# jbikker/tinybvh

Measured on AMD Instinct MI355X. Metric: MRays/s (primary + diffuse) on Bistro CWBVH, higher is better.
Workload: dtype f32; 1 GPU; procedural street (Bistro-exterior stand-in, 2.83M tris, seed 2); BVH8_CWBVH; per GPU per step 16777216 primary + 16777216 diffuse (depth 1-3) Intersect; scene_tris=2832120, layout=BVH8_CWBVH, scene_is_stand_in=True

## Files before the change

### include/tinybvh_amd.h

```cpp
#ifndef TINYBVH_AMD_H_
#define TINYBVH_AMD_H_

#include <stddef.h>
#include <stdint.h>

#ifdef __cplusplus
extern "C" {
#endif

#define TBVH_ABI_VERSION 5

#define TBVH_OK            0
#define TBVH_E_INVALID    -1
#define TBVH_E_NODEVICE   -2
#define TBVH_E_HIP        -3
#define TBVH_E_NOMEM      -4
#define TBVH_E_FORMAT     -5

#define TBVH_LAYOUT_BVH2_WALD  1
#define TBVH_LAYOUT_BVH_DOUBLE 3
#define TBVH_LAYOUT_BVH_GPU    5
#define TBVH_LAYOUT_BVH4_GPU   8
#define TBVH_LAYOUT_CWBVH     10
#define TBVH_LAYOUT_VOXELSET  12

typedef struct tbvh_context tbvh_context;
typedef struct tbvh_scene   tbvh_scene;
typedef struct tbvh_hostbvh tbvh_hostbvh;

int         tbvh_abi_version(void);
const char* tbvh_last_error(void);
int         tbvh_device_count(void);
int         tbvh_init(int device, tbvh_context** out);
void        tbvh_shutdown(tbvh_context* ctx);
int         tbvh_synchronize(tbvh_context* ctx);
int         tbvh_set_stream(tbvh_context* ctx, void* hip_stream);
int         tbvh_set_timing(tbvh_context* ctx, int enabled);


int tbvh_upload_bvh_gpu(tbvh_context* ctx, const void* nodes64, uint64_t n_nodes,
                        const uint32_t* prim_idx, uint64_t n_idx,
                        const void* verts16, uint64_t n_tris, tbvh_scene** out);

int tbvh_upload_bvh4_gpu(tbvh_context* ctx, const void* blocks16, uint64_t n_blocks,
                         tbvh_scene** out);

int tbvh_upload_cwbvh(tbvh_context* ctx, const void* nodes16, uint64_t n_node_blocks,
                      const void* tris16, uint64_t n_tri_blocks, tbvh_scene** out);

int tbvh_upload_tlas(tbvh_context* ctx, const void* tlas_nodes64, uint64_t n_nodes,
                     const uint32_t* tlas_idx, uint64_t n_idx,
                     const void* instances192, uint64_t n_instances,
                     tbvh_scene* const* blas, uint64_t n_blas, tbvh_scene** out);
int tbvh_update_tlas(tbvh_scene* tlas, const void* tlas_nodes64, uint64_t n_nodes,
                     const uint32_t* tlas_idx, uint64_t n_idx,
                     const void* instances192, uint64_t n_instances);

int tbvh_update_bvh_gpu(tbvh_scene* scene, const void* nodes64, uint64_t n_nodes, const uint32_t* prim_idx, uint64_t n_idx, const void* verts16, uint64_t n_tris);
int tbvh_update_bvh4_gpu(tbvh_scene* scene, const void* blocks16, uint64_t n_blocks);
int tbvh_update_cwbvh(tbvh_scene* scene, const void* nodes16, uint64_t n_node_blocks, const void* tris16, uint64_t n_tri_blocks);

int tbvh_convert_bvh2_device(tbvh_context* ctx, const void* nodes32, uint64_t n_nodes, const uint32_t* prim_idx, uint64_t n_idx,
                             const void* verts16, uint64_t n_tris, int on_device, int layout, tbvh_scene** out);

int tbvh_build_device(tbvh_context* ctx, const void* verts16, uint64_t n_tris, int on_device, int layout,
                      uint32_t max_leaf_tris, tbvh_scene** out);

int tbvh_build_device_ploc(tbvh_context* ctx, const void* verts16, uint64_t n_tris, int on_device, int layout, uint32_t radius, tbvh_scene** out);

int tbvh_scene_download(tbvh_scene* scene, int which, void* dst, uint64_t cap_bytes, uint64_t* bytes_out);

int tbvh_set_opacity_micromaps(tbvh_scene* blas, const uint32_t* map_data, uint32_t N, uint64_t n_tris, int on_device);

int tbvh_refit(tbvh_scene* scene, const void* verts16, uint64_t n_tris, int on_device);

int tbvh_rebuild_tlas_device(tbvh_scene* tlas, const void* transforms, int on_device,
                             const float* blas_bounds6, uint64_t n_blas);
int tbvh_tlas_download(tbvh_scene* tlas, void* tlas_nodes64, uint64_t cap_nodes, uint32_t* tlas_idx, uint64_t cap_idx,
                       void* instances192, uint64_t cap_instances, uint64_t* n_nodes_out);
void     tbvh_free_scene(tbvh_scene* scene);
int      tbvh_scene_layout(const tbvh_scene* scene);
uint64_t tbvh_scene_device_bytes(const tbvh_scene* scene);


int tbvh_intersect(tbvh_scene* scene, void* rays, uint64_t n_rays, uint32_t stride_bytes);
int tbvh_occluded(tbvh_scene* scene, const void* rays, uint64_t n_rays,
                  uint32_t stride_bytes, uint8_t* occluded);
int tbvh_pinned_malloc(tbvh_context* ctx, uint64_t bytes, void** out);
int tbvh_pinned_free(tbvh_context* ctx, void* ptr);

int tbvh_intersect_device(tbvh_scene* scene, void* d_rays64, uint64_t n_rays);
int tbvh_occluded_device(tbvh_scene* scene, const void* d_rays64, uint64_t n_rays,
                         uint8_t* d_occluded);
int tbvh_intersect_device_fresh(tbvh_scene* scene, void* d_rays64, uint64_t n_rays, float tmax);

int tbvh_intersect_sharded(tbvh_scene* const* scenes, uint32_t n_devices, void* rays, uint64_t n_rays, uint32_t stride_bytes);
int tbvh_occluded_sharded(tbvh_scene* const* scenes, uint32_t n_devices, const void* rays, uint64_t n_rays,
                          uint32_t stride_bytes, uint8_t* occluded);
int tbvh_intersect_sharded_device(tbvh_scene* const* scenes, uint32_t n_devices, void* const* d_rays64, const uint64_t* n_rays,
                                  int fresh, float tmax, float* kernel_ms, float* dispatch_ms);
int tbvh_occluded_sharded_device(tbvh_scene* const* scenes, uint32_t n_devices, const void* const* d_rays64, const uint64_t* n_rays,
                                 uint8_t* const* d_occluded, float* kernel_ms, float* dispatch_ms);
void tbvh_shard_range(uint64_t n_rays, uint32_t rank, uint32_t world, uint64_t* begin, uint64_t* end);

int tbvh_reset_hits_device(tbvh_context* ctx, void* d_rays64, uint64_t n_rays, float tmax);

float tbvh_time_last_ms(tbvh_context* ctx);

int tbvh_time_history(tbvh_context* ctx, float* ms, uint32_t cap, uint32_t* count);

int tbvh_measure_copy_bandwidth(tbvh_context* ctx, uint64_t bytes, uint32_t reps, double* gbps);
int tbvh_measure_read_bandwidth(tbvh_context* ctx, uint64_t bytes, uint32_t reps, double* gbps);
int tbvh_measure_valu_issue(tbvh_context* ctx, uint32_t reps, double* ginstr_per_s);
int tbvh_measure_link_bandwidth(tbvh_context* ctx, uint64_t bytes, uint32_t reps, double* h2d_gbps, double* d2h_gbps);

int tbvh_cwbvh_set_hybrid(tbvh_scene* scene, int64_t packed_nodes);

typedef struct tbvh_schedule_hint { uint8_t closest_hit[3]; uint8_t any_hit[3]; uint8_t reserved[2]; } tbvh_schedule_hint;
int tbvh_scene_get_schedule_hint(tbvh_scene* scene, tbvh_schedule_hint* out);
// ... 289 lines not shown
```

### include/tinybvh_amd_debug.h

```cpp
#ifndef TINYBVH_AMD_DEBUG_H_
#define TINYBVH_AMD_DEBUG_H_
#include "tinybvh_amd.h"
#ifdef __cplusplus
extern "C" {
#endif

int tbvh_debug_stats(tbvh_context* ctx, uint64_t out[8], int reset);

int tbvh_debug_set_flags(tbvh_context* ctx, uint32_t flags);

int tbvh_debug_coherent_schedule(tbvh_scene* scene, int anyhit, uint32_t out[4]);

int tbvh_debug_last_probe(tbvh_context* ctx, uint32_t out[3]);

int tbvh_set_variant(tbvh_scene* scene, int variant);

int tbvh_debug_wide_copy_bvh2(int layout, const void* blob, uint64_t n_blob, const uint32_t* prim_idx, uint64_t n_idx, const void* verts16, uint64_t n_tris,
                              uint32_t max_leaf_tris, void* nodes32_out, uint64_t cap_nodes, uint64_t* n_nodes_out, void* recs_out, uint64_t cap_recs,
                              uint64_t* n_recs_out);

int tbvh_debug_device_allocations(uint64_t out[2]);

struct tbvh_scenegraph;
int tbvh_debug_scenegraph_array(struct tbvh_scenegraph* g, int what, void** d_ptr);
int tbvh_debug_scenegraph_step(struct tbvh_scenegraph* g, int step, float dt);
struct tbvh_host_scenegraph;
int tbvh_debug_host_scenegraph_set_trs(struct tbvh_host_scenegraph* g, const float* trs10, uint64_t n_nodes);
int tbvh_debug_host_scenegraph_check_chains(struct tbvh_host_scenegraph* g, uint64_t* n_differ);

#ifdef __cplusplus
}
#endif
#endif
```

### tinybvh_amd/__init__.py

```python
from __future__ import annotations

import ctypes as C
from typing import Optional

import os

import numpy as np

from . import _capi
from ._capi import AlphaTexture, BuildParams, Camera, Mesh, OmmSource, TbvhError, check, lib

LAYOUT_BVH2_WALD = 1
LAYOUT_BVH_DOUBLE = 3
LAYOUT_BVH_GPU = 5
LAYOUT_BVH4_GPU = 8
LAYOUT_CWBVH = 10
LAYOUT_VOXELSET = 12
MATERIAL_DIFFUSE, MATERIAL_LIGHT, MATERIAL_SPECULAR = 0, 1, 2

BVH_FAR = np.float32(1e30)

RAY_DTYPE = np.dtype([
    ("O", "<f4", 3), ("mask", "<u4"),
    ("D", "<f4", 3), ("instIdx", "<u4"),
    ("rD", "<f4", 3), ("inst", "<u4"),
    ("t", "<f4"), ("u", "<f4"), ("v", "<f4"), ("prim", "<u4"),
])
assert RAY_DTYPE.itemsize == 64


def safercp(x: np.ndarray) -> np.ndarray:
    x = np.asarray(x, dtype=np.float32)
    big = np.abs(x) > np.float32(1e-12)
    with np.errstate(divide="ignore"):
        r = np.where(big, np.float32(1.0) / np.where(big, x, np.float32(1.0)), np.where(x >= 0, BVH_FAR, -BVH_FAR))
    return r.astype(np.float32)


def make_rays(O: np.ndarray, D: np.ndarray, tmax=BVH_FAR, normalize: bool = True) -> np.ndarray:
    O = np.ascontiguousarray(O, dtype=np.float32).reshape(-1, 3)
    D = np.ascontiguousarray(D, dtype=np.float32).reshape(-1, 3)
    if normalize:
        l = np.sqrt((D * D).sum(axis=1, dtype=np.float32)).astype(np.float32)
        rl = np.where(l == 0, np.float32(0), np.float32(1) / np.where(l == 0, np.float32(1), l)).astype(np.float32)
        D = (D * rl[:, None]).astype(np.float32)
    rays = np.zeros(O.shape[0], dtype=RAY_DTYPE)
    rays["O"] = O
    rays["D"] = D
    rays["rD"] = safercp(D)
    rays["mask"] = 0xFFFF
    rays["t"] = tmax
    return rays


def _ptr(a: np.ndarray) -> C.c_void_p:
    return C.c_void_p(a.ctypes.data)


class Context:

    def __init__(self, device: int = 0):
        h = C.c_void_p()
        check(lib.tbvh_init(device, C.byref(h)), "tbvh_init")
        self._h = h
        self.device = device

    def close(self):
        if self._h:
            lib.tbvh_shutdown(self._h)
            self._h = None

    def __del__(self):
        try:
            self.close()
        except Exception:
            pass

    def synchronize(self):
        check(lib.tbvh_synchronize(self._h), "tbvh_synchronize")

    def set_stream(self, hip_stream: Optional[int]):
        check(lib.tbvh_set_stream(self._h, C.c_void_p(hip_stream or 0)), "tbvh_set_stream")

    def set_timing(self, enabled: bool):
        check(lib.tbvh_set_timing(self._h, 1 if enabled else 0), "tbvh_set_timing")

    def copy_bandwidth_gbps(self, nbytes: int = 1 << 30, reps: int = 3) -> float:
        g = C.c_double(0)
        check(lib.tbvh_measure_copy_bandwidth(self._h, nbytes, reps, C.byref(g)), "tbvh_measure_copy_bandwidth")
        return float(g.value)

    def read_bandwidth_gbps(self, nbytes: int = 1 << 30, reps: int = 3) -> float:
        g = C.c_double(0)
        check(lib.tbvh_measure_read_bandwidth(self._h, nbytes, reps, C.byref(g)), "tbvh_measure_read_bandwidth")
        return float(g.value)

    def valu_issue_ginstr(self, reps: int = 3) -> float:
        g = C.c_double(0)
        check(lib.tbvh_measure_valu_issue(self._h, reps, C.byref(g)), "tbvh_measure_valu_issue")
        return float(g.value)

    def link_bandwidth_gbps(self, nbytes: int = 1 << 28, reps: int = 3):
        up, down = C.c_double(0), C.c_double(0)
        check(lib.tbvh_measure_link_bandwidth(self._h, nbytes, reps, C.byref(up), C.byref(down)), "tbvh_measure_link_bandwidth")
        return float(up.value), float(down.value)

    def pinned_array(self, shape, dtype) -> np.ndarray:
        dt = np.dtype(dtype)
        n = int(np.prod(shape)) * dt.itemsize
        p = C.c_void_p()
        check(lib.tbvh_pinned_malloc(self._h, max(n, 1), C.byref(p)), "tbvh_pinned_malloc")
        buf = (C.c_char * max(n, 1)).from_address(p.value)
        a = np.frombuffer(buf, dtype=dt, count=int(np.prod(shape))).reshape(shape)
        self._pinned = getattr(self, "_pinned", {})
        self._pinned[a.ctypes.data] = p.value
        return a

    def pinned_free(self, a: np.ndarray):
        p = getattr(self, "_pinned", {}).pop(a.ctypes.data, None)
        check(lib.tbvh_pinned_free(self._h, C.c_void_p(p if p is not None else a.ctypes.data)), "tbvh_pinned_free")

    def time_last_ms(self) -> float:
        return float(lib.tbvh_time_last_ms(self._h))

    def time_history(self, k: int):
        buf = (C.c_float * max(int(k), 1))()
        cnt = C.c_uint32(0)
        check(lib.tbvh_time_history(self._h, buf, int(k), C.byref(cnt)), "tbvh_time_history")
        return [float(buf[i]) for i in range(cnt.value)]

    def set_debug_flags(self, flags: int):
        check(lib.tbvh_debug_set_flags(self._h, int(flags)), "tbvh_debug_set_flags")

    def last_probe(self):
        out = (C.c_uint32 * 3)()
        check(lib.tbvh_debug_last_probe(self._h, out), "tbvh_debug_last_probe")
        return int(out[0]), int(out[1]), int(out[2])

    def malloc(self, nbytes: int) -> int:
        p = C.c_void_p()
        check(lib.tbvh_device_malloc(self._h, nbytes, C.byref(p)), "tbvh_device_malloc")
        return p.value

    def free(self, dptr: int):
        check(lib.tbvh_device_free(self._h, C.c_void_p(dptr)), "tbvh_device_free")

    def to_device(self, dptr: int, a: np.ndarray):
        a = np.ascontiguousarray(a)
        check(lib.tbvh_copy_to_device(self._h, C.c_void_p(dptr), _ptr(a), a.nbytes), "tbvh_copy_to_device")

    def from_device(self, a: np.ndarray, dptr: int):
        assert a.flags["C_CONTIGUOUS"]
        check(lib.tbvh_copy_from_device(self._h, _ptr(a), C.c_void_p(dptr), a.nbytes), "tbvh_copy_from_device")

    def flatten_mesh(self, verts, indices=None, d_out: int = 0) -> int:
        m, keep = _mesh(verts, indices)
        d = d_out or self.malloc(int(m.n_tris) * 48)
        check(lib.tbvh_flatten_mesh_device(self._h, C.byref(m), C.c_void_p(d)), "tbvh_flatten_mesh_device")
        return d

    def reset_hits(self, d_rays: int, n: int, tmax: float = 1e30):
        check(lib.tbvh_reset_hits_device(self._h, C.c_void_p(d_rays), n, float(tmax)), "tbvh_reset_hits_device")

    def generate_primary(self, cam: Camera, d_rays: int, first: int, n: int):
        check(lib.tbvh_generate_primary_device(self._h, C.byref(cam), C.c_void_p(d_rays), first, n), "tbvh_generate_primary_device")
# ... 1469 lines not shown
```

### tinybvh_amd/_capi.py

```python
from __future__ import annotations

import ctypes as C
import os

_HERE = os.path.dirname(os.path.abspath(__file__))
LIB_PATH = os.environ.get("TBVH_LIB_OVERRIDE") or os.path.join(_HERE, "libtinybvh_amd.so")

_u64, _u32, _vp, _i = C.c_uint64, C.c_uint32, C.c_void_p, C.c_int
_pp = C.POINTER(C.c_void_p)


class BuildParams(C.Structure):
    _fields_ = [("bins", _u32), ("max_leaf_tris", _u32), ("threads", _u32), ("flags", _u32)]


class Mesh(C.Structure):
    _fields_ = [("verts", C.c_void_p), ("n_verts", C.c_uint64), ("stride_bytes", C.c_uint32), ("on_device", C.c_uint32),
                ("indices", C.c_void_p), ("n_tris", C.c_uint64)]


class AlphaTexture(C.Structure):
    _fields_ = [("texels", C.c_void_p), ("width", C.c_uint32), ("height", C.c_uint32)]


class OmmSource(C.Structure):
    _fields_ = [("uv", C.c_void_p), ("n_uv", C.c_uint64), ("uv_stride_bytes", C.c_uint32), ("on_device", C.c_uint32), ("indices", C.c_void_p),
                ("n_tris", C.c_uint64), ("tri_texture", C.c_void_p), ("textures", C.POINTER(AlphaTexture)), ("n_textures", C.c_uint32)]


class SceneGraphDesc(C.Structure):
    _fields_ = [("flags", C.c_uint32), ("n_nodes", C.c_uint64), ("parent", C.c_void_p), ("visit_order", C.c_void_p), ("translation", C.c_void_p), ("rotation", C.c_void_p),
                ("scale", C.c_void_p), ("matrix", C.c_void_p), ("local_transform", C.c_void_p), ("n_weights", C.c_void_p), ("weights", C.c_void_p),
                ("n_samplers", C.c_uint64), ("sampler_interpolation", C.c_void_p), ("sampler_type", C.c_void_p), ("sampler_key_offset", C.c_void_p),
                ("sampler_value_offset", C.c_void_p), ("key_times", C.c_void_p), ("key_values", C.c_void_p), ("n_animations", C.c_uint64), ("n_channels", C.c_uint64),
                ("channel_animation", C.c_void_p), ("channel_sampler", C.c_void_p), ("channel_node", C.c_void_p), ("channel_target", C.c_void_p),
                ("n_instances", C.c_uint64), ("node_of_instance", C.c_void_p), ("n_skin_uses", C.c_uint64), ("skin_mesh_node", C.c_void_p),
                ("skin_joint_offset", C.c_void_p), ("skin_joint_node", C.c_void_p), ("skin_inverse_bind", C.c_void_p)]


class Camera(C.Structure):
    _fields_ = [("eye", C.c_float * 3), ("p1", C.c_float * 3), ("p2", C.c_float * 3), ("p3", C.c_float * 3),
                ("width", _u32), ("height", _u32), ("spp_x", _u32), ("spp_y", _u32)]


class WfParams(C.Structure):
    _fields_ = [("light_pos", C.c_float * 3), ("light_color", C.c_float * 3), ("sky_lo", C.c_float * 3), ("sky_hi", C.c_float * 3),
                ("eps", C.c_float), ("max_depth", _u32), ("seed", _u32), ("clear", _u32), ("light_size", C.c_float * 2), ("flags", _u32), ("sample_index", _u32)]


class WfStats(C.Structure):
    _fields_ = [("extend_rays", _u64 * 8), ("shadow_rays", _u64 * 8), ("frame_ms", C.c_float)]


SYMBOLS = {
    "tbvh_debug_wide_copy_bvh2": (_i, [_i, _vp, _u64, _vp, _u64, _vp, _u64, _u32, _vp, _u64, C.POINTER(_u64), _vp, _u64, C.POINTER(_u64)]),
    "tbvh_wavefront_create": (_i, [_vp, _u32, _u32, _pp]),
    "tbvh_wavefront_destroy": (None, [_vp]),
    "tbvh_wavefront_render": (_i, [_vp, _vp, _vp, C.POINTER(Camera), C.POINTER(WfParams), C.POINTER(WfStats)]),
    "tbvh_wavefront_read": (_i, [_vp, _vp]),
    "tbvh_wavefront_set_blas_vertices": (_i, [_vp, _vp, _u64]),
    "tbvh_wavefront_finalize": (_i, [_vp, C.c_float, _vp]),
    "tbvh_wavefront_set_blue_noise": (_i, [_vp, _vp, _u64]),
    "tbvh_abi_version": (_i, []),
    "tbvh_last_error": (C.c_char_p, []),
    "tbvh_device_count": (_i, []),
    "tbvh_init": (_i, [_i, _pp]),
    "tbvh_shutdown": (None, [_vp]),
    "tbvh_synchronize": (_i, [_vp]),
    "tbvh_set_stream": (_i, [_vp, _vp]),
    "tbvh_set_timing": (_i, [_vp, _i]),
    "tbvh_upload_bvh_gpu": (_i, [_vp, _vp, _u64, _vp, _u64, _vp, _u64, _pp]),
    "tbvh_upload_bvh4_gpu": (_i, [_vp, _vp, _u64, _pp]),
    "tbvh_upload_cwbvh": (_i, [_vp, _vp, _u64, _vp, _u64, _pp]),
    "tbvh_upload_tlas": (_i, [_vp, _vp, _u64, _vp, _u64, _vp, _u64, _pp, _u64, _pp]),
    "tbvh_update_tlas": (_i, [_vp, _vp, _u64, _vp, _u64, _vp, _u64]),
    "tbvh_update_bvh_gpu": (_i, [_vp, _vp, _u64, _vp, _u64, _vp, _u64]),
    "tbvh_update_bvh4_gpu": (_i, [_vp, _vp, _u64]),
    "tbvh_update_cwbvh": (_i, [_vp, _vp, _u64, _vp, _u64]),
    "tbvh_rebuild_tlas_device": (_i, [_vp, _vp, _i, _vp, _u64]),
    "tbvh_refit": (_i, [_vp, _vp, _u64, _i]),
    "tbvh_set_opacity_micromaps": (_i, [_vp, _vp, _u32, _u64, _i]),
    "tbvh_scene_download": (_i, [_vp, _i, _vp, _u64, _vp]),
    "tbvh_build_device": (_i, [_vp, _vp, _u64, _i, _i, _u32, _vp]),
    "tbvh_build_device_ploc": (_i, [_vp, _vp, _u64, _i, _i, _u32, _vp]),
    "tbvh_convert_bvh2_device": (_i, [_vp, _vp, _u64, _vp, _u64, _vp, _u64, _i, _i, _vp]),
    "tbvh_tlas_download": (_i, [_vp, _vp, _u64, _vp, _u64, _vp, _u64, _vp]),
    "tbvh_free_scene": (None, [_vp]),
    "tbvh_scene_layout": (_i, [_vp]),
    "tbvh_scene_device_bytes": (_u64, [_vp]),
    "tbvh_intersect": (_i, [_vp, _vp, _u64, _u32]),
    "tbvh_occluded": (_i, [_vp, _vp, _u64, _u32, _vp]),
    "tbvh_intersect_sharded": (_i, [_vp, _u32, _vp, _u64, _u32]),
    "tbvh_occluded_sharded": (_i, [_vp, _u32, _vp, _u64, _u32, _vp]),
    "tbvh_intersect_sharded_device": (_i, [_vp, _u32, _vp, _vp, _i, C.c_float, _vp, _vp]),
    "tbvh_occluded_sharded_device": (_i, [_vp, _u32, _vp, _vp, _vp, _vp, _vp]),
    "tbvh_wavefront_set_band": (_i, [_vp, _u32, _u32]),
    "tbvh_wavefront_render_sharded": (_i, [_vp, _vp, _vp, _u32, C.POINTER(Camera), _vp, _vp, _vp]),
    "tbvh_wavefront_read_sharded": (_i, [_vp, _u32, _vp]),
    "tbvh_shard_range": (None, [_u64, _u32, _u32, C.POINTER(_u64), C.POINTER(_u64)]),
    "tbvh_intersect_device": (_i, [_vp, _vp, _u64]),
    "tbvh_occluded_device": (_i, [_vp, _vp, _u64, _vp]),
    "tbvh_intersect_device_fresh": (_i, [_vp, _vp, _u64, C.c_float]),
    "tbvh_reset_hits_device": (_i, [_vp, _vp, _u64, C.c_float]),
    "tbvh_time_last_ms": (C.c_float, [_vp]),
    "tbvh_debug_coherent_schedule": (C.c_int, [_vp, C.c_int, C.POINTER(C.c_uint32)]),
    "tbvh_time_history": (C.c_int, [_vp, C.POINTER(C.c_float), C.c_uint32, C.POINTER(C.c_uint32)]),
    "tbvh_measure_copy_bandwidth": (_i, [_vp, _u64, _u32, C.POINTER(C.c_double)]),
    "tbvh_measure_read_bandwidth": (_i, [_vp, _u64, _u32, C.POINTER(C.c_double)]),
    "tbvh_measure_valu_issue": (_i, [_vp, _u32, C.POINTER(C.c_double)]),
    "tbvh_measure_link_bandwidth": (_i, [_vp, _u64, _u32, C.POINTER(C.c_double), C.POINTER(C.c_double)]),
    "tbvh_scene_get_schedule_hint": (_i, [_vp, _vp]),
    "tbvh_scene_set_schedule_hint": (_i, [_vp, _vp]),
    "tbvh_pinned_malloc": (_i, [_vp, _u64, _pp]),
    "tbvh_pinned_free": (_i, [_vp, _vp]),
    "tbvh_set_variant": (_i, [_vp, _i]),
    "tbvh_debug_stats": (_i, [_vp, _vp, _i]),
    "tbvh_debug_last_probe": (_i, [_vp, _vp]),
    "tbvh_debug_set_flags": (_i, [_vp, _u32]),
    "tbvh_debug_device_allocations": (_i, [C.POINTER(_u64)]),
    "tbvh_cwbvh_set_hybrid": (_i, [_vp, C.c_int64]),
    "tbvh_bin_rays_device": (_i, [_vp, _vp, _vp, _u64, C.POINTER(C.c_float), _u32, _u32, _vp]),
    "tbvh_generate_primary_device": (_i, [_vp, C.POINTER(Camera), _vp, _u64, _u64]),
    "tbvh_generate_bounce_device": (_i, [_vp, _vp, _vp, _vp, _u64, _u32]),
    "tbvh_generate_shadow_device": (_i, [_vp, _vp, _vp, _u64, C.POINTER(C.c_float), C.c_float]),
    "tbvh_device_malloc": (_i, [_vp, _u64, _pp]),
    "tbvh_device_free": (_i, [_vp, _vp]),
    "tbvh_copy_to_device": (_i, [_vp, _vp, _vp, _u64]),
    "tbvh_copy_from_device": (_i, [_vp, _vp, _vp, _u64]),
    "tbvh_host_build": (_i, [_vp, _u64, _i, C.POINTER(BuildParams), _pp]),
    "tbvh_host_build_tlas": (_i, [_vp, _u64, _vp, _u64, _pp]),
    "tbvh_host_free": (None, [_vp]),
    "tbvh_cwbvh_file_write": (_i, [C.c_char_p, _vp, _u64, _vp, _u64, _u64, _vp]),
    "tbvh_cwbvh_file_read": (_i, [C.c_char_p, _u64, _pp, C.POINTER(_u64)]),
    "tbvh_host_layout": (_i, [_vp]),
    "tbvh_host_blob": (_vp, [_vp, _i]),
    "tbvh_host_blob_count": (_u64, [_vp, _i]),
    "tbvh_upload_host": (_i, [_vp, _vp, _vp, _u64, _pp]),
    "tbvh_upload_bvh_double": (_i, [_vp, _vp, _u64, _vp, _u64, _vp, _u64, _pp]),
    "tbvh_upload_tlas_double": (_i, [_vp, _vp, _u64, _vp, _u64, _vp, _u64, _pp, _u64, _pp]),
    "tbvh_intersect_ex_device": (_i, [_vp, _vp, _u64]),
    "tbvh_occluded_ex_device": (_i, [_vp, _vp, _u64, _vp]),
    "tbvh_intersect_ex": (_i, [_vp, _vp, _u64]),
    "tbvh_occluded_ex": (_i, [_vp, _vp, _u64, _vp]),
    "tbvh_host_build_double": (_i, [_vp, _u64, _pp]),
    "tbvh_host_build_tlas_double": (_i, [_vp, _u64, _vp, _u64, _pp]),
    "tbvh_rebuild_tlas_double_device": (_i, [_vp, _vp, _i]),
    "tbvh_update_tlas_double": (_i, [_vp, _vp, _u64, _vp, _u64, _vp, _u64]),
    "tbvh_tlas_double_download": (_i, [_vp, _vp, _u64, _vp, _u64, _vp, _u64, _vp]),
    "tbvh_double_download": (_i, [_vp, _vp, _u64, _vp]),
    "tbvh_refit_double": (_i, [_vp, _vp, _u64, _i]),
    "tbvh_upload_voxelset": (_i, [_vp, _vp, _vp, _u64, _vp, _pp]),
    "tbvh_host_build_voxelset": (_i, [_vp, _u32, _u32, _u32, _pp]),
# ... 105 lines not shown
```

### tinybvh_amd/csrc/capi_context.hip

```cpp
#include "capi_internal.h"

using namespace tbvh;
using namespace tbvh_capi;

namespace {
thread_local char g_err[512] = "";
}

namespace tbvh_capi {
int fail(int code, const char* fmt, ...) {
    va_list ap;
    va_start(ap, fmt);
    vsnprintf(g_err, sizeof g_err, fmt, ap);
    va_end(ap);
    return code;
}

int setDevice(tbvh_context* c) {
    HIP_TRY(hipSetDevice(c->device));
    return 0;
}
hipError_t timedBegin(tbvh_context* c) {
    if (c->skipTiming) return hipSuccess;
    const uint32_t slot = (uint32_t)(c->evSeq % tbvh_context::kTimeRing);
    for (int k = 0; k < 2; k++)
        if (!c->evRing[slot][k]) { const hipError_t e = hipEventCreate(&c->evRing[slot][k]); if (e != hipSuccess) return e; }
    c->evDone[slot] = false;
    c->ev0 = c->evRing[slot][0]; c->ev1 = c->evRing[slot][1];
    c->evSeq++;
    return hipEventRecord(c->ev0, c->stream);
}
hipError_t timedEnd(tbvh_context* c) {
    if (c->skipTiming) return hipSuccess;
    const hipError_t e = hipEventRecord(c->ev1, c->stream);
    if (e == hipSuccess && c->evSeq) { c->evDone[(c->evSeq - 1) % tbvh_context::kTimeRing] = true; c->timed = true; }
    return e;
}
}

extern "C" {

int tbvh_abi_version(void) { return TBVH_ABI_VERSION; }
const char* tbvh_last_error(void) { return g_err; }

int tbvh_device_count(void) {
    int n = 0;
    hipError_t e = hipGetDeviceCount(&n);
    if (e != hipSuccess) { fail(TBVH_E_HIP, "hipGetDeviceCount: %s", hipGetErrorString(e)); return e == hipErrorNoDevice ? 0 : TBVH_E_HIP; }
    return n;
}

int tbvh_init(int device, tbvh_context** out) {
    if (!out) return fail(TBVH_E_INVALID, "tbvh_init: out is null");
    *out = nullptr;
    int n = 0;
    if (hipGetDeviceCount(&n) != hipSuccess || n <= 0) return fail(TBVH_E_NODEVICE, "no HIP device available");
    if (device < 0 || device >= n) return fail(TBVH_E_NODEVICE, "device %d out of range (0..%d)", device, n - 1);
    tbvh_context* c = new (std::nothrow) tbvh_context;
    if (!c) return fail(TBVH_E_NOMEM, "out of host memory");
    c->device = device;
    hipDeviceProp_t prop;
    hipError_t e = hipSetDevice(device);
    if (e == hipSuccess) e = hipGetDeviceProperties(&prop, device);
    if (e == hipSuccess) e = hipStreamCreateWithFlags(&c->ownStream, hipStreamNonBlocking);
    if (e != hipSuccess) { delete c; return fail(TBVH_E_HIP, "context setup failed: %s", hipGetErrorString(e)); }
    c->stream = c->ownStream;
    c->numCUs = prop.multiProcessorCount;
    c->blocks = (uint32_t)c->numCUs * 24u;
    if (const char* e = getenv("TBVH_BLOCKS_PER_CU")) {
        const int b = atoi(e);
        if (b >= 1 && b <= 32) { c->blocks = (uint32_t)c->numCUs * (uint32_t)b; c->gridOverride = true; }
    }
    if (const char* e = getenv("TBVH_RAYS_PER_BLOCK")) {
        const int b = atoi(e);
        if (b >= 64 && b <= 4096) { c->raysPerBlock = (uint32_t)b; c->gridOverride = true; }
    }
    if (const char* e = getenv("TBVH_SPLIT_RAYS")) { if (atoi(e) == 0) c->splitBelow = 0; }
    if (const char* e = getenv("TBVH_INCOHERENT_COPIES")) { if (atoi(e) == 0) c->incoherentCopies = false; }
    if (const char* e = getenv("TBVH_EMBED_TRIS")) { if (atoi(e) == 0) c->embedTris = false; }
    if (const char* e = getenv("TBVH_DEBUG_FLAGS")) c->expFlags = (uint32_t)strtoul(e, nullptr, 0);
    if (const char* e = getenv("TBVH_COHERENT_TUNER")) { const int v = atoi(e); c->cohTunerMode = v == 0 ? 1 : (v == 2 ? 2 : (v == 3 ? 3 : 0)); }
    if (const char* e = getenv("TBVH_POOL_PARTS")) {
        const int b = atoi(e);
        if (b >= 0 && (1 << b) <= kPoolParts) c->poolParts = (uint32_t)b;
    }
    c->spillEntries = 232;
    if (const char* e2 = getenv("TBVH_SPILL_ENTRIES")) {
        const int v = atoi(e2);
        if (v >= 2 && v <= 232) c->spillEntries = (uint32_t)v & ~1u;
    }
    const size_t spillBytes = (size_t)(c->blocks + c->blocks / 3u) * 64 * c->spillEntries * 4;
    e = c->spill.alloc(spillBytes / 4);
    if (e == hipSuccess) e = c->counter.alloc(32);
    if (e == hipSuccess) e = c->pool.alloc((size_t)(kPoolParts + 1) * kPoolCounterStride * 2);
    if (e != hipSuccess) { tbvh_shutdown(c); return fail(TBVH_E_NOMEM, "device allocation failed: %s", hipGetErrorString(e)); }
    c->status = (uint32_t*)(c->counter.get() + 4);
    hipMemset(c->counter, 0, 256);
    *out = c;
    return 0;
}

void tbvh_shutdown(tbvh_context* c) {
    if (!c) return;
    hipSetDevice(c->device);
    if (c->ownStream) hipStreamSynchronize(c->ownStream);
    for (;;) {
        tbvh_scene* t = nullptr;
        for (tbvh_scene* s : c->scenes) if (s->isTlas) { t = s; break; }
        if (!t) break;
        tbvh_free_scene(t);
    }
    while (!c->scenes.empty()) tbvh_free_scene(c->scenes.back());
    freePosesOf(c);
    freeGraphsOf(c);
    freeShadingsOf(c);
    freeOmmStagingOf(c);
    for (const tbvh_context::PinnedRange& r : c->pinned) hipHostFree(r.host);
    c->pinned.clear();
    delete c->pipe;
    for (auto& pair : c->evRing) for (hipEvent_t ev : pair) if (ev) hipEventDestroy(ev);
    if (c->ownStream) hipStreamDestroy(c->ownStream);
    delete c;
}

int tbvh_debug_device_allocations(uint64_t out[2]) {
    if (!out) return fail(TBVH_E_INVALID, "tbvh_debug_device_allocations: null argument");
    out[0] = g_devBufLive.load(); out[1] = g_devBufBytes.load();
    return 0;
}

int tbvh_synchronize(tbvh_context* c) {
    if (!c) return fail(TBVH_E_INVALID, "null context");
    TBVH_ENTER(c);
    HIP_TRY(hipStreamSynchronize(c->stream));
    return 0;
}

int tbvh_set_stream(tbvh_context* c, void* s) {
    if (!c) return fail(TBVH_E_INVALID, "null context");
    TBVH_LOCK(c);
    c->stream = s ? (hipStream_t)s : c->ownStream;
    return 0;
}

float tbvh_time_last_ms(tbvh_context* c) {
    if (!c) return -1.0f;
    TBVH_LOCK(c);
    if (!c->timed) return -1.0f;
    if (c->hostQuerySeq == c->evSeq && c->hostQueryMs >= 0.f) return c->hostQueryMs;
    hipSetDevice(c->device);
    if (hipEventSynchronize(c->ev1) != hipSuccess) return -1.0f;
    float ms = -1.0f;
    if (hipEventElapsedTime(&ms, c->ev0, c->ev1) != hipSuccess) return -1.0f;
    return ms;
}

int tbvh_time_history(tbvh_context* c, float* ms, uint32_t cap, uint32_t* count) {
    if (!c || !count || (!ms && cap)) return fail(TBVH_E_INVALID, "tbvh_time_history: null argument");
    *count = 0;
    TBVH_ENTER(c);
    uint64_t n = c->evSeq < tbvh_context::kTimeRing ? c->evSeq : tbvh_context::kTimeRing;
    if (n > cap) n = cap;
    for (uint64_t i = 0; i < n; i++) {
        const uint32_t slot = (uint32_t)((c->evSeq - n + i) % tbvh_context::kTimeRing);
        float t = -1.0f;
        if (c->evDone[slot]) {
            HIP_TRY(hipEventSynchronize(c->evRing[slot][1]));
            HIP_TRY(hipEventElapsedTime(&t, c->evRing[slot][0], c->evRing[slot][1]));
        }
        ms[i] = t;
    }
    *count = (uint32_t)n;
    return 0;
}

int tbvh_debug_stats(tbvh_context* c, uint64_t out[8], int reset) {
    if (!c || !out) return fail(TBVH_E_INVALID, "tbvh_debug_stats: null argument");
    TBVH_ENTER(c);
    HIP_TRY(hipStreamSynchronize(c->stream));
    HIP_TRY(hipMemcpy(out, c->counter + 8, 64, hipMemcpyDeviceToHost));
    if (reset) HIP_TRY(hipMemset(c->counter + 8, 0, 64));
    return 0;
}

int tbvh_set_timing(tbvh_context* c, int enabled) {
    if (!c) return fail(TBVH_E_INVALID, "tbvh_set_timing: null context");
    TBVH_LOCK(c);
    c->skipTiming = enabled == 0;
    return 0;
}

int tbvh_debug_set_flags(tbvh_context* c, uint32_t flags) {
    if (!c) return fail(TBVH_E_INVALID, "tbvh_debug_set_flags: null context");
    TBVH_LOCK(c);
    c->expFlags = flags;
    return 0;
}

int tbvh_debug_last_probe(tbvh_context* c, uint32_t out[3]) {
    if (!c || !out) return fail(TBVH_E_INVALID, "tbvh_debug_last_probe: null argument");
    TBVH_ENTER(c);
    out[0] = out[1] = out[2] = 0;
    if (!c->lastProbed) return 0;
    HIP_TRY(hipStreamSynchronize(c->stream));
    HIP_TRY(hipMemcpy(out, (uint32_t*)c->pool + (size_t)(c->poolCur ^ 1) * ((size_t)(kPoolParts + 1) * kPoolCounterStride) + (size_t)kPoolParts * kPoolCounterStride, 8, hipMemcpyDeviceToHost));
    out[2] = (out[1] != 0 && out[0] * 10u >= out[1] * 6u) ? 2u : 1u;
    return 0;
}


int tbvh_device_malloc(tbvh_context* c, uint64_t bytes, void** out) {
    if (!c || !out) return fail(TBVH_E_INVALID, "tbvh_device_malloc: null argument");
    TBVH_ENTER(c);
    hipError_t e = hipMalloc(out, bytes ? bytes : 16);
    if (e != hipSuccess) return fail(TBVH_E_NOMEM, "hipMalloc(%llu): %s", (unsigned long long)bytes, hipGetErrorString(e));
    return 0;
}
int tbvh_device_free(tbvh_context* c, void* p) {
    if (!c) return fail(TBVH_E_INVALID, "null context");
    TBVH_ENTER(c);
    HIP_TRY(hipStreamSynchronize(c->stream));
    HIP_TRY(hipFree(p));
    return 0;
}
int tbvh_copy_to_device(tbvh_context* c, void* d, const void* src, uint64_t bytes) {
    if (!c || ((!d || !src) && bytes)) return fail(TBVH_E_INVALID, "tbvh_copy_to_device: null argument");
    TBVH_ENTER(c);
    HIP_TRY(hipMemcpyAsync(d, src, bytes, hipMemcpyHostToDevice, c->stream));
    HIP_TRY(hipStreamSynchronize(c->stream));
    return 0;
}
int tbvh_copy_from_device(tbvh_context* c, void* dst, const void* d, uint64_t bytes) {
    if (!c || ((!d || !dst) && bytes)) return fail(TBVH_E_INVALID, "tbvh_copy_from_device: null argument");
    TBVH_ENTER(c);
    HIP_TRY(hipMemcpyAsync(dst, d, bytes, hipMemcpyDeviceToHost, c->stream));
    HIP_TRY(hipStreamSynchronize(c->stream));
    return 0;
}

static int timeBest(tbvh_context* c, uint32_t reps, const std::function<void()>& launch, double* bestMs) {
    hipEvent_t e0 = nullptr, e1 = nullptr;
    HIP_TRY(hipEventCreate(&e0));
    if (hipEventCreate(&e1) != hipSuccess) { hipEventDestroy(e0); return fail(TBVH_E_HIP, "hipEventCreate failed"); }
    double best = 0;
    hipError_t err = hipSuccess;
    for (uint32_t i = 0; i <= reps && err == hipSuccess; i++) {
        err = hipEventRecord(e0, c->stream);
        launch();
        if (err == hipSuccess) err = hipGetLastError();
        if (err == hipSuccess) err = hipEventRecord(e1, c->stream);
        if (err == hipSuccess) err = hipEventSynchronize(e1);
        float ms = 0;
        if (err == hipSuccess) err = hipEventElapsedTime(&ms, e0, e1);
        if (err == hipSuccess && i && ms > 0 && (best == 0 || ms < best)) best = ms;
    }
    hipEventDestroy(e0); hipEventDestroy(e1);
    if (err != hipSuccess) return fail(TBVH_E_HIP, "measurement launch failed: %s", hipGetErrorString(err));
    if (best <= 0) return fail(TBVH_E_HIP, "measurement produced no timing");
    *bestMs = best;
    return 0;
}

int tbvh_measure_copy_bandwidth(tbvh_context* c, uint64_t bytes, uint32_t reps, double* gbps) {
    if (!c || !gbps || bytes < (1u << 20)) return fail(TBVH_E_INVALID, "tbvh_measure_copy_bandwidth: null argument or under 1 MB");
    TBVH_ENTER(c);
    DevBuf<void> a, b;
    if (a.alloc(bytes) != hipSuccess || b.alloc(bytes) != hipSuccess) return fail(TBVH_E_NOMEM, "tbvh_measure_copy_bandwidth: cannot allocate 2 x %llu bytes", (unsigned long long)bytes);
    int r = 0;
    if (hipMemsetAsync(a, 1, bytes, c->stream) != hipSuccess) r = fail(TBVH_E_HIP, "hipMemsetAsync failed");
    double ms = 0;
    if (!r) r = timeBest(c, reps ? reps : 3, [&] { launch_stream_copy((const float4*)a.get(), (float4*)b.get(), bytes / 16, c->stream); }, &ms);
    if (r) return r;
    *gbps = 2.0 * (double)bytes / (ms * 1e-3) / 1e9;
    return 0;
}

int tbvh_measure_read_bandwidth(tbvh_context* c, uint64_t bytes, uint32_t reps, double* gbps) {
    if (!c || !gbps || bytes < (1u << 20)) return fail(TBVH_E_INVALID, "tbvh_measure_read_bandwidth: null argument or under 1 MB");
    TBVH_ENTER(c);
    DevBuf<void> a;
    DevBuf<float> sink;
    if (a.alloc(bytes) != hipSuccess || sink.alloc(64) != hipSuccess) return fail(TBVH_E_NOMEM, "tbvh_measure_read_bandwidth: cannot allocate %llu bytes", (unsigned long long)bytes);
    int r = 0;
    if (hipMemsetAsync(a, 1, bytes, c->stream) != hipSuccess) r = fail(TBVH_E_HIP, "hipMemsetAsync failed");
    double ms = 0;
    if (!r) r = timeBest(c, reps ? reps : 3, [&] { launch_stream_read((const float4*)a.get(), sink, bytes / 16, (uint32_t)c->numCUs * 32u, c->stream); }, &ms);
    if (r) return r;
    *gbps = (double)bytes / (ms * 1e-3) / 1e9;
// ... 36 lines not shown
```

### tinybvh_amd/csrc/capi_internal.h

```cpp
#pragma once
#include "../../include/tinybvh_amd.h"
#include "../../include/tinybvh_amd_debug.h"

#include <hip/hip_runtime.h>

#include <chrono>
#include <cmath>
#include <cstdarg>
#include <cstdio>
#include <cstdlib>
#include <cstring>
#include <new>
#include <atomic>
#include <condition_variable>
#include <functional>
#include <memory>
#include <mutex>
#include <string>
#include <thread>
#include <vector>

#include "copy_policy.h"
#include "dev_buf.h"
#include "host_builder.h"
#include "kernels.h"
#include "ray_pool.h"

using namespace tbvh;
using tbvh_capi::DevBuf;
using tbvh_capi::CopyKind;
using tbvh_capi::CopyPolicy;
using tbvh_capi::kCopyWide4;
using tbvh_capi::kCopyWide8;

static_assert(kLayoutBvhGpu == TBVH_LAYOUT_BVH_GPU && kLayoutBvh4Gpu == TBVH_LAYOUT_BVH4_GPU && kLayoutCwbvh == TBVH_LAYOUT_CWBVH,
              "kernels.h and the public header agree on the layout codes");

namespace tbvh_capi {
int fail(int code, const char* fmt, ...);
}

#define TBVH_REFUSE_DOUBLE(scene, who)                                                                                              \
    do {                                                                                                                            \
        if ((scene) && (scene)->layout == TBVH_LAYOUT_BVH_DOUBLE)                                                                   \
            return tbvh_capi::fail(TBVH_E_INVALID, "%s: a BVH_DOUBLE scene takes tbvh_intersect_ex / tbvh_occluded_ex only", who);   \
    } while (0)

#define TBVH_REFUSE_VOXEL(scene, who)                                                                                                   \
    do {                                                                                                                                \
        if ((scene) && (scene)->layout == TBVH_LAYOUT_VOXELSET)                                                                         \
            return tbvh_capi::fail(TBVH_E_INVALID, "%s: a VOXELSET scene takes the queries and can be a TLAS's BLAS; nothing else", who); \
    } while (0)

#define TBVH_REFUSE_CUSTOM(scene, who)                                                                                                    \
    do {                                                                                                                                  \
        if ((scene) && (scene)->layout == TBVH_LAYOUT_BVH2_WALD)                                                                          \
            return tbvh_capi::fail(TBVH_E_INVALID, "%s: a sphere BLAS (custom geometry) takes the queries and can be a TLAS's BLAS; nothing else", who); \
    } while (0)

#define HIP_TRY(expr)                                                                        \
    do {                                                                                     \
        hipError_t e_ = (expr);                                                              \
        if (e_ != hipSuccess) return fail(TBVH_E_HIP, "%s failed: %s", #expr, hipGetErrorString(e_)); \
    } while (0)

struct tbvh_context {
    std::recursive_mutex mu;
    int device = 0;
    hipStream_t ownStream = nullptr;
    hipStream_t stream = nullptr;
    static constexpr uint32_t kTimeRing = 256;
    hipEvent_t evRing[kTimeRing][2] = {};
    bool evDone[kTimeRing] = {};
    int cohTunerMode = 0;
    uint64_t evSeq = 0;
    hipEvent_t ev0 = nullptr, ev1 = nullptr;
    bool timed = false;
    int numCUs = 0;
    uint32_t blocks = 0;
    DevBuf<uint32_t> spill;
    uint32_t spillEntries = 0;
    DevBuf<unsigned long long> counter;
    uint32_t poolParts = 5;
    bool embedTris = true;
    bool incoherentCopies = true;
    uint32_t expFlags = 0;
    bool skipTiming = false;
    bool lastProbed = false;
    bool gridOverride = false;
    uint64_t splitBelow = 12ull << 20;
    uint32_t raysPerBlock = 128;
    DevBuf<uint32_t> pool;
    int poolCur = 0;
    bool poolClean = false;
    uint32_t* status = nullptr;
    DevBuf<RayRec> stageRays;
    DevBuf<uint8_t> stageOcc;
    struct HostPipe* pipe = nullptr;
    struct PinnedRange { char* host; uint64_t bytes; };
    float hostQueryMs = -1.f;
    uint64_t hostQuerySeq = ~0ull;
    std::vector<PinnedRange> pinned;
    DevBuf<void> binScratch;
    std::vector<tbvh_scene*> scenes;
    std::vector<struct tbvh_pose*> poses;
    std::vector<struct tbvh_scenegraph*> graphs;
    std::vector<struct tbvh_shading*> shadings;
    DevBuf<void> ommDesc;
    void* ommPin = nullptr;
    size_t ommPinBytes = 0;
    hipEvent_t ommEv = nullptr;
    bool ommPinUsed = false;
};

struct CohTuner {
    int decided = 0;
    bool pinned = false;
    uint32_t launches = 0;
    uint64_t refRays = 0;
    static constexpr int kModes = 3;
    uint32_t n[kModes] = {0, 0, 0};
    float best[kModes] = {1e30f, 1e30f, 1e30f};
    struct Pending { hipEvent_t e0, e1; int mode; uint64_t rays; };
    std::vector<Pending> pending;
    static constexpr uint32_t kSamples = 3;
    void drop_pending() { for (Pending& p : pending) { hipEventDestroy(p.e0); hipEventDestroy(p.e1); } pending.clear(); }
    void harvest(float minMs);
    void settle(bool packetOrStrict, float margin);
    int least_sampled() const;
};

struct WideCopies {
    tbvh_scene* copy8 = nullptr;
    tbvh_scene* copy4 = nullptr;
    bool tried8 = false, tried4 = false;
    bool tlasOnly = false;
    CopyPolicy policy;
    uint8_t live() const { return (uint8_t)((copy8 ? kCopyWide8 : 0) | (copy4 ? kCopyWide4 : 0)); }
    uint8_t pending() const { return policy.pendingCopies; }
};

struct CwbvhLayouts {
    DevBuf<float4> padded;
    DevBuf<float4> hybrid;
    DevBuf<uint32_t> perm;
    DevBuf<float4> trisPadded;
    uint32_t packed = 0;
    bool tried = false;
    bool levelOrder = false;
};

struct tbvh_scene {
    tbvh_context* ctx = nullptr;
    int layout = 0;
    int variant = 0;
    DevBuf<float4> nodes;
    DevBuf<float4> tris;
    CwbvhLayouts cw;
    CohTuner cohTuner[2][4];
    uint8_t cohLastClass[2] = {2, 2};
    uint32_t nNodes = 0;
    uint64_t nNodeBlocks = 0, nTriBlocks = 0;
    uint64_t capNodeBlocks = 0, capTriBlocks = 0;
    uint64_t topoHash = 0;
    uint64_t bytes = 0;
    bool isTlas = false;
    DevBuf<uint32_t> tlasIdx;
    DevBuf<float4> instances;
    DevBuf<BlasDesc> blasDesc;
    int blasLayout = 0;
    bool blasMixCw2 = false;
    bool blasSpheres = false;
    DevBuf<BlasDesc> blasDescAny;
    bool anyHitSeen = false;
    int blasLayoutAny = -1;
    bool blasMixCw2Any = false;
    uint64_t nInst = 0, nBlas = 0, nTlasNodes = 0, nTlasIdx = 0;
    DevBuf<float4> tlas4;
// ... 30 lines not shown
    uint64_t dblTris = 0, dblRecs = 0;
    uint32_t dblLeaves = 0;
};

struct BLASInstanceCheck { float m[32]; float mn[3]; uint32_t blasIdx; float mx[3]; uint32_t mask; uint32_t pad[8]; };
static_assert(sizeof(BLASInstanceCheck) == 192, "BLASInstance is 192 bytes");

struct tbvh_hostbvh {
    int layout = 0;
    BVH2 bvh2;
    std::vector<NodeAL> al;
    std::vector<Vec4> blocksA, blocksB;
    std::vector<NodeDbl> dnodes;
    std::vector<uint64_t> didx;
    std::vector<uint32_t> vgrid, vbricks, vtop;
};

struct HostPipe {
    static constexpr uint64_t kChunk = 1ull << 18;
    void* pinUp[2] = {nullptr, nullptr};
    hipEvent_t evUp[2] = {nullptr, nullptr};
    hipStream_t down = nullptr;
    hipEvent_t evKernel = nullptr;
    std::vector<hipEvent_t> evGroup;
    DevBuf<uint32_t> packed;
    void* pinDown = nullptr;
    std::vector<std::thread> workers;
    std::mutex m;
    std::condition_variable cvWork, cvDone;
    std::function<void(uint32_t, uint32_t)> job;
    uint64_t generation = 0;
    uint32_t pending = 0;
    bool quit = false;
    void start(uint32_t nThreads) {
        for (uint32_t t = 0; t < nThreads; t++)
            workers.emplace_back([this, t, nThreads] {
                uint64_t seen = 0;
                for (;;) {
                    std::function<void(uint32_t, uint32_t)> f;
                    {
                        std::unique_lock<std::mutex> lk(m);
                        cvWork.wait(lk, [&] { return quit || generation != seen; });
                        if (quit) return;
                        seen = generation; f = job;
                    }
                    f(t + 1, nThreads + 1);
                    {
                        std::lock_guard<std::mutex> lk(m);
                        if (--pending == 0) cvDone.notify_all();
                    }
                }
            });
    }
    void parallel_for(uint64_t items, const std::function<void(uint32_t, uint32_t)>& f) {
        if (items < 16384 || workers.empty()) { f(0, 1); return; }
        {
            std::lock_guard<std::mutex> lk(m);
            job = f; pending = (uint32_t)workers.size(); generation++;
        }
        cvWork.notify_all();
        f(0, (uint32_t)workers.size() + 1);
        std::unique_lock<std::mutex> lk(m);
        cvDone.wait(lk, [&] { return pending == 0; });
    }
    ~HostPipe() {
        { std::lock_guard<std::mutex> lk(m); quit = true; }
        cvWork.notify_all();
        for (auto& w : workers) w.join();
        for (int i = 0; i < 2; i++) {
            if (pinUp[i]) hipHostFree(pinUp[i]);
            if (evUp[i]) hipEventDestroy(evUp[i]);
        }
        for (hipEvent_t e : evGroup) hipEventDestroy(e);
        if (evKernel) hipEventDestroy(evKernel);
        if (down) hipStreamDestroy(down);
        if (pinDown) hipHostFree(pinDown);
    }
};

namespace tbvh_capi {
int setDevice(tbvh_context* c);
#define TBVH_LOCK(ctxptr) std::lock_guard<std::recursive_mutex> ctx_lock_((ctxptr)->mu)
#define TBVH_ENTER(ctxptr) std::lock_guard<std::recursive_mutex> ctx_lock_((ctxptr)->mu); if (int r_ = tbvh_capi::setDevice(ctxptr)) return r_
hipError_t timedBegin(tbvh_context* c);
hipError_t timedEnd(tbvh_context* c);
int launchQuery(tbvh_scene* s, tbvh::RayRec* d_rays, uint64_t n, uint8_t* d_occ, bool fresh = false, float freshTmax = 1e30f,
                const unsigned long long* nDev = nullptr);
int checkStatus(tbvh_context* c);
int ensureStage(tbvh_context* c, uint64_t n);
int ensureStageOcc(tbvh_context* c, uint64_t n);
tbvh_scene* newScene(tbvh_context* c, int layout);
int reclassifyTlas(tbvh_scene* t);
uint64_t cwbvhTopologyHash(const tbvh::Vec4* nodes, uint32_t nNodes);
int prepareIncoherentCopies(tbvh_scene* s);
int rederiveCwbvhLayouts(tbvh_scene* s);
int resetCwbvhLayouts(tbvh_scene* s, bool levelOrder = false);
void freeCopy(tbvh_scene* s, CopyKind kind);
void makeCopyOnce(tbvh_scene* b, CopyKind kind);
void dropCopiesAfterUpdate(tbvh_scene* s);
void countQueryForRecopy(tbvh_scene* s);
tbvh_scene* wideCopyForQuery(tbvh_scene* s);
tbvh_scene* tunedScene(tbvh_scene* s);
void shareOpacityMaps(tbvh_scene* s);
int refitCopies(tbvh_scene* s, const tbvh::MeshSrc& src);
const tbvh_scene* blasView(const tbvh_scene* b, bool any, bool allow4 = true);
template <class F>
int forEachTlasOver(tbvh_scene* b, F f) {
    for (size_t i = 0; i < b->usedBy.size(); i++) {
        bool seen = false;
        for (size_t k = 0; k < i; k++) seen |= b->usedBy[k] == b->usedBy[i];
        if (!seen) if (int r = f(b->usedBy[i])) return r;
    }
    return 0;
}
int checkMesh(const tbvh_mesh* m, const char* who, bool indicesMayBeHeld = false);
tbvh_mesh flatMesh(const void* verts16, uint64_t nTris, int onDevice);
uint64_t meshVertexBytes(const tbvh_mesh& m);
struct DeviceMesh {
    tbvh::MeshSrc src;
    DevBuf<void> ownVerts;
    DevBuf<uint32_t> ownIdx;
};
int stageMesh(tbvh_context* c, const tbvh_mesh& m, DeviceMesh& out);
int keepMeshIndices(tbvh_scene* s, const tbvh::MeshSrc& src);
int convertDeviceImpl(tbvh_context* c, int layout, const float4* dN2, uint64_t nNodes2, const uint32_t* dIdx, uint64_t nIdx, const tbvh::MeshSrc& dV, tbvh_scene** out);
int refitDeviceSource(tbvh_scene* s, const tbvh::MeshSrc& src);
int hostBuildImpl(const tbvh::HostMesh& mesh, uint64_t nTris, int layout, const tbvh_build_params* p, tbvh_hostbvh** out);
int checkSphereScene(tbvh_scene* s, const char* who);
int launchSpheres(tbvh_scene* s, const float4* dSpheres, uint64_t n, const tbvh::MeshSrc& verts, uint8_t* dHit);
int allocOpacityMaps(tbvh_context* c, uint32_t N, uint64_t nTris, const char* who, DevBuf<uint32_t>& fresh, uint64_t* wordsOut);
int installOpacityMaps(tbvh_scene* s, DevBuf<uint32_t>&& fresh, uint32_t N);
void freeOmmStagingOf(tbvh_context* c);
void freeGraphsOf(tbvh_context* c);
void freePosesOf(tbvh_context* c);
void freeShadingsOf(tbvh_context* c);
tbvh_context* shadingContext(const struct tbvh_shading* sh);
void shadingSlotRecords(const struct tbvh_shading* sh, uint32_t slot, float4** tris, uint64_t* nTris);
void detachPosesFrom(tbvh_context* c, const struct tbvh_shading* sh);
}
```

### tinybvh_amd/csrc/capi_pose.hip

```cpp
#include "capi_internal.h"
#include "pose.h"

using namespace tbvh;
using namespace tbvh_capi;

struct tbvh_pose {
    tbvh_context* ctx = nullptr;
    int kind = 0;
    uint64_t nVerts = 0;
    uint32_t nJoints = 0, nTargets = 0;
    DevBuf<float4> rest, weights;
    DevBuf<uint4> joints;
    DevBuf<float> positions;
    DevBuf<float> params;
    DevBuf<float4> out;
    tbvh_shading* shading = nullptr;
    uint32_t slot = 0;
    uint64_t fatTris = 0;
    DevBuf<float> normals;
    DevBuf<float4> nOut;
    DevBuf<uint32_t> fatIdx;
    char* pin = nullptr;
    uint64_t pinSlotBytes = 0;
    hipEvent_t pinEv[2] = {nullptr, nullptr};
// ... 151 lines not shown
    if (nTargets != p->nTargets) return fail(TBVH_E_INVALID, "tbvh_pose_set_morph: %u weights, the pose was created with %u targets", nTargets, p->nTargets);
    if (nTargets && !weights) return fail(TBVH_E_INVALID, "tbvh_pose_set_morph: null weights");
    if (onDevice && ((uintptr_t)weights & 3)) return fail(TBVH_E_INVALID, "tbvh_pose_set_morph: device weights must be 4-byte aligned");
    tbvh_context* c = p->ctx;
    TBVH_ENTER(c);
    float4* fat = nullptr;
    if (int r = attachedRecords(p, "tbvh_pose_set_morph", &fat)) return r;
    const float* dW = nullptr;
    if (int r = stageParams(p, weights, (uint64_t)nTargets * 4, onDevice, &dW)) return r;
    HIP_TRY(timedBegin(c));
    if (p->shading) {
        launch_pose_morph_normals(p->positions, nTargets ? dW : p->params.get(), nTargets, p->normals, p->out, p->nOut, p->nVerts, c->stream);
        updateFatTris(p, fat);
    } else
        launch_pose_morph(p->positions, nTargets ? dW : p->params.get(), nTargets, p->out, p->nVerts, c->stream);
    HIP_TRY(hipGetLastError());
    HIP_TRY(timedEnd(c));
    return 0;
}

int tbvh_pose_attach_fat_tris(tbvh_pose* p, tbvh_shading* sh, uint32_t slot, const float* normals12, const uint32_t* indices, uint64_t nTris, int onDevice) {
    if (!p || !sh || !normals12) return fail(TBVH_E_INVALID, "tbvh_pose_attach_fat_tris: null argument");
    if (shadingContext(sh) != p->ctx) return fail(TBVH_E_INVALID, "tbvh_pose_attach_fat_tris: the pose and the shading table belong to different contexts");
    if (((uintptr_t)normals12 | (uintptr_t)indices) & 3) return fail(TBVH_E_INVALID, "tbvh_pose_attach_fat_tris: misaligned normals or indices (4 bytes)");
    if (nTris == 0 || nTris >> 32) return fail(TBVH_E_INVALID, "tbvh_pose_attach_fat_tris: %llu triangles", (unsigned long long)nTris);
    if (!indices && p->nVerts != 3 * nTris)
        return fail(TBVH_E_INVALID, "tbvh_pose_attach_fat_tris: %llu vertices for %llu triangles: without indices triangle i has corners 3i .. 3i + 2", (unsigned long long)p->nVerts, (unsigned long long)nTris);
    tbvh_context* c = p->ctx;
    TBVH_ENTER(c);
    float4* tris = nullptr; uint64_t have = 0;
    shadingSlotRecords(sh, slot, &tris, &have);
    if (have != nTris) return fail(TBVH_E_INVALID, "tbvh_pose_attach_fat_tris: slot %u of the shading table holds %llu records, not %llu", slot, (unsigned long long)have, (unsigned long long)nTris);
    if (indices && !onDevice) {
        const uint64_t bad = pose_first_bad_corner(indices, nTris, p->nVerts);
        if (bad != nTris) return fail(TBVH_E_FORMAT, "tbvh_pose_attach_fat_tris: triangle %llu: an index is not a vertex (%llu vertices)", (unsigned long long)bad, (unsigned long long)p->nVerts);
    }
    const uint64_t nFloats = (p->kind == kPoseMorph ? (uint64_t)p->nTargets + 1 : 1) * p->nVerts * 3;
    DevBuf<float> normals; DevBuf<float4> nOut; DevBuf<uint32_t> idx;
    if (normals.alloc(nFloats) != hipSuccess || nOut.alloc(p->nVerts) != hipSuccess || (indices && idx.alloc(3 * nTris) != hipSuccess))
        return allocFail("tbvh_pose_attach_fat_tris", nFloats * 4 + p->nVerts * 16 + (indices ? nTris * 12 : 0));
    const hipMemcpyKind kind = onDevice ? hipMemcpyDeviceToDevice : hipMemcpyHostToDevice;
    HIP_TRY(hipMemcpyAsync(normals, normals12, nFloats * 4, kind, c->stream));
    if (indices) HIP_TRY(hipMemcpyAsync(idx, indices, nTris * 12, kind, c->stream));
    HIP_TRY(hipStreamSynchronize(c->stream));
    p->normals = std::move(normals); p->nOut = std::move(nOut); p->fatIdx = std::move(idx);
    p->shading = sh; p->slot = slot; p->fatTris = nTris;
    return 0;
}

int tbvh_pose_vertices(tbvh_pose* p, const void** dVerts16, uint64_t* nVerts) {
    if (!p || !dVerts16) return fail(TBVH_E_INVALID, "tbvh_pose_vertices: null argument");
    TBVH_LOCK(p->ctx);
    *dVerts16 = p->out.get();
    if (nVerts) *nVerts = p->nVerts;
    return 0;
}

int tbvh_pose_refit(tbvh_pose* p, tbvh_scene* s) {
    if (!p || !s) return fail(TBVH_E_INVALID, "tbvh_pose_refit: null argument");
    if (s->ctx != p->ctx) return fail(TBVH_E_INVALID, "tbvh_pose_refit: the pose and the scene belong to different contexts");
    TBVH_ENTER(p->ctx);
    if (s->meshIdx) {
        tbvh_mesh m;
        m.verts = p->out.get(); m.n_verts = p->nVerts; m.stride_bytes = 16; m.on_device = 1; m.indices = nullptr; m.n_tris = s->meshIdxTris;
        return tbvh_refit_mesh(s, &m);
    }
    if (p->nVerts % 3) return fail(TBVH_E_INVALID, "tbvh_pose_refit: %llu vertices: a scene without an index buffer takes 3 per triangle", (unsigned long long)p->nVerts);
    return tbvh_refit(s, p->out.get(), p->nVerts / 3, 1);
}

int tbvh_pose_download(tbvh_pose* p, void* dst16, uint64_t capVerts) {
    if (!p || !dst16) return fail(TBVH_E_INVALID, "tbvh_pose_download: null argument");
    if (capVerts < p->nVerts) return fail(TBVH_E_INVALID, "tbvh_pose_download: room for %llu vertices, the pose has %llu", (unsigned long long)capVerts, (unsigned long long)p->nVerts);
    tbvh_context* c = p->ctx;
    TBVH_ENTER(c);
    HIP_TRY(hipMemcpyAsync(dst16, p->out, p->nVerts * 16, hipMemcpyDeviceToHost, c->stream));
    return checkStatus(c);
}

void tbvh_pose_free(tbvh_pose* p) {
    if (!p) return;
    tbvh_context* c = p->ctx;
    TBVH_LOCK(c);
    hipSetDevice(c->device);
    hipStreamSynchronize(c->stream);
    for (size_t i = 0; i < c->poses.size(); i++)
        if (c->poses[i] == p) { c->poses.erase(c->poses.begin() + i); break; }
    destroyPose(p);
}

}
```

### tinybvh_amd/csrc/capi_query.hip

```cpp
#include "capi_internal.h"

using namespace tbvh;
using namespace tbvh_capi;

namespace tbvh_capi {
int ensureStage(tbvh_context* c, uint64_t n) {
    HIP_TRY(c->stageRays.reserve(n));
    return 0;
}
int ensureStageOcc(tbvh_context* c, uint64_t n) {
    HIP_TRY(c->stageOcc.reserve(n));
    return 0;
}
}

void CohTuner::harvest(float minMs) {
    for (size_t k = 0; k < pending.size();) {
        const Pending pe = pending[k];
        const hipError_t qe = hipEventQuery(pe.e1);
        if (qe == hipErrorNotReady) { (void)hipGetLastError(); k++; continue; }
        float t1 = 0.f;
        if (qe == hipSuccess && hipEventElapsedTime(&t1, pe.e0, pe.e1) == hipSuccess && t1 > minMs) {
            if (!refRays) refRays = pe.rays;
            if (pe.rays * 4 >= refRays * 3 && pe.rays * 3 <= refRays * 4) {
// ... 69 lines not shown
constexpr uint64_t kDirectRays = 16384;

static int hostQuerySmall(tbvh_scene* s, const char* raysIn, char* raysOut, uint64_t n, uint32_t stride, uint8_t* occ) {
    tbvh_context* c = s->ctx;
    if (int r = ensureStage(c, n)) return r;
    if (occ) if (int r = ensureStageOcc(c, n)) return r;
    HIP_TRY(hipMemcpy2DAsync(c->stageRays, 64, raysIn, stride, 64, n, hipMemcpyHostToDevice, c->stream));
    if (int r = launchQuery(s, c->stageRays, n, occ ? c->stageOcc : nullptr)) return r;
    if (occ) HIP_TRY(hipMemcpyAsync(occ, c->stageOcc, n, hipMemcpyDeviceToHost, c->stream));
    else HIP_TRY(hipMemcpy2DAsync(raysOut + 44, stride, (const char*)c->stageRays.get() + 44, 64, 20, n, hipMemcpyDeviceToHost, c->stream));
    return checkStatus(c);
}

int hostQuery(tbvh_scene* s, const char* raysIn, char* raysOut, uint64_t n, uint32_t stride, uint8_t* occ) {
    tbvh_context* c = s->ctx;
    if (n <= kDirectRays) return hostQuerySmall(s, raysIn, raysOut, n, stride, occ);
    if (int r = ensureStage(c, n)) return r;
    if (occ) if (int r = ensureStageOcc(c, n)) return r;
    const uint64_t G = n <= kGroupRays + kGroupRays / 2 ? 1 : (n + kGroupRays - 1) / kGroupRays;
    const uint64_t per = (((n + G - 1) / G) + HostPipe::kChunk - 1) / HostPipe::kChunk * HostPipe::kChunk;
    if (int r = ensurePipe(c, occ ? (n + 19) / 20 : 2 * per)) return r;
    HostPipe* p = c->pipe;
    const bool direct = stride == 64 && isPinned(c, raysIn, n * 64);
    while (p->evGroup.size() < G) { hipEvent_t e = nullptr; HIP_TRY(hipEventCreateWithFlags(&e, hipEventDisableTiming)); p->evGroup.push_back(e); }
    const uint64_t seq0 = c->evSeq;
    uint64_t chunkNo = 0;
    auto drain = [&](uint64_t g) -> int {
        const uint64_t b = g * per, e = b + per < n ? b + per : n;
        HIP_TRY(hipEventSynchronize(p->evGroup[g]));
        const char* pin = (const char*)p->pinDown + (g & 1) * per * 20;
        p->parallel_for(e - b, [=](uint32_t part, uint32_t parts) {
            const uint64_t lo = (e - b) * part / parts, hi = (e - b) * (part + 1) / parts;
            for (uint64_t i = lo; i < hi; i++) std::memcpy(raysOut + (b + i) * stride + 44, pin + i * 20, 20);
        });
        return 0;
    };
    for (uint64_t g = 0; g < G; g++) {
        const uint64_t b = g * per, e = b + per < n ? b + per : n;
        for (uint64_t first = b; first < e; first += HostPipe::kChunk, chunkNo++) {
            const uint64_t cnt = e - first < HostPipe::kChunk ? e - first : HostPipe::kChunk;
            if (direct) { HIP_TRY(hipMemcpyAsync(c->stageRays + first, raysIn + first * 64, cnt * 64, hipMemcpyHostToDevice, c->stream)); continue; }
            const int k = (int)(chunkNo & 1);
            if (chunkNo >= 2) HIP_TRY(hipEventSynchronize(p->evUp[k]));
            char* pin = (char*)p->pinUp[k];
            const char* src = raysIn + first * stride;
            p->parallel_for(cnt, [=](uint32_t part, uint32_t parts) {
                const uint64_t lo = cnt * part / parts, hi = cnt * (part + 1) / parts;
                if (stride == 64) std::memcpy(pin + lo * 64, src + lo * 64, (hi - lo) * 64);
                else for (uint64_t i = lo; i < hi; i++) std::memcpy(pin + i * 64, src + i * stride, 64);
            });
            HIP_TRY(hipMemcpyAsync(c->stageRays + first, pin, cnt * 64, hipMemcpyHostToDevice, c->stream));
            HIP_TRY(hipEventRecord(p->evUp[k], c->stream));
        }
        if (int r = launchQuery(s, c->stageRays + b, e - b, occ ? c->stageOcc + b : nullptr)) return r;
        if (!occ) {
            uint32_t* packed = p->packed + (g & 1) * per * 5;
            HIP_TRY(hipEventRecord(p->evKernel, c->stream));
            HIP_TRY(hipStreamWaitEvent(p->down, p->evKernel, 0));
            launch_pack_hits(c->stageRays + b, packed, e - b, p->down);
            HIP_TRY(hipGetLastError());
            HIP_TRY(hipMemcpyAsync((char*)p->pinDown + (g & 1) * per * 20, packed, (e - b) * 20, hipMemcpyDeviceToHost, p->down));
            HIP_TRY(hipEventRecord(p->evGroup[g], p->down));
            if (g) if (int r = drain(g - 1)) return r;
        }
    }
    if (occ) HIP_TRY(hipMemcpyAsync(p->pinDown, c->stageOcc, n, hipMemcpyDeviceToHost, c->stream));
    else if (int r = drain(G - 1)) return r;
    if (int r = checkStatus(c)) return r;
    if (occ) std::memcpy(occ, p->pinDown, n);
    if (!c->skipTiming && c->evSeq - seq0 == G && G <= tbvh_context::kTimeRing) {
        float sum = 0.f; bool ok = true;
        for (uint64_t q = seq0; q < c->evSeq && ok; q++) {
            const uint32_t slot = (uint32_t)(q % tbvh_context::kTimeRing);
            float t = 0.f;
            ok = c->evDone[slot] && hipEventElapsedTime(&t, c->evRing[slot][0], c->evRing[slot][1]) == hipSuccess;
            sum += t;
        }
        if (ok) { c->hostQueryMs = sum; c->hostQuerySeq = c->evSeq; } else (void)hipGetLastError();
    }
    return 0;
}


static void launchTlasKernels(tbvh_scene* s, QueryArgs& q, bool any, uint32_t blocks) {
    tbvh_context* c = s->ctx;
    const uint32_t blocks7 = (!c->gridOverride && blocks == c->blocks) ? (uint32_t)c->numCUs * 28u : blocks;
    const bool own = any && s->blasDescAny != nullptr;
    const int layout = own ? s->blasLayoutAny : s->blasLayout;
    const bool mix = own ? s->blasMixCw2Any : s->blasMixCw2;
    const BlasDesc* desc = own ? s->blasDescAny : s->blasDesc;
    if (s->blasSpheres) {
        q.spillStride = c->spillEntries / 2;
        launch_tlas_custom(any, layout, s->nodes, s->tlasIdx, s->instances, desc, q, c->status, blocks, c->stream);
    } else if (s->tlas4 && layout == TBVH_LAYOUT_BVH4_GPU) {
        q.spillStride = c->spillEntries;
        launch_tlas4(any, 0, s->tlas4, s->instances, desc, q, c->status, blocks, c->stream, blocks7);
    } else if (s->tlas8 && (layout == TBVH_LAYOUT_CWBVH || mix)) {
        q.spillStride = c->spillEntries / 2;
        launch_tlas8(any, 0, s->tlas8, s->tlas8Refs, s->instances, desc, q, c->status, blocks, c->stream, blocks7, mix);
    } else if (layout == TBVH_LAYOUT_VOXELSET) {
        q.spillStride = c->spillEntries;
        launch_voxel(any, nullptr, s->nodes, s->tlasIdx, s->instances, desc, q, c->status, blocks, c->stream);
    } else if (layout == TBVH_LAYOUT_BVH_GPU) {
        q.spillStride = c->spillEntries;
        launch_tlas2(any, 0, s->nodes, s->tlasIdx, s->instances, desc, q, c->status, blocks, c->stream, blocks7);
    } else {
        q.spillStride = c->spillEntries / 2;
        launch_tlas(any, layout, s->nodes, s->tlasIdx, s->instances, desc, q, c->status, blocks, c->stream);
    }
}

struct CwbvhLaunch {
    bool any;
    bool small;
    bool probedSmall;
    int sizeClass;
    uint32_t blocks;
    uint32_t blocksBase;
    uint32_t* probeWords;
};

static int launchCoherentFlavor(tbvh_scene* s, const QueryArgs& q, const CwbvhLaunch& L, const float4* tris, uint32_t blocks7) {
    tbvh_context* c = s->ctx;
    QueryArgs qa = q;
    qa.baseBlocks = 0;
    if (c->expFlags & 16u) qa.flags |= 16u;
    s->cohLastClass[L.any ? 1 : 0] = (uint8_t)L.sizeClass;
    CohTuner& tu = s->cohTuner[L.any ? 1 : 0][L.sizeClass];
    const bool sizeKnown = q.nRaysDev == nullptr;
    if (L.probedSmall && !tu.decided && tu.n[0] == 0) { tu.n[0] = CohTuner::kSamples; tu.best[0] = 1e30f; }
    if (!tu.decided && !c->cohTunerMode) {
        tu.harvest(L.probedSmall ? 0.015f : 0.05f);
        tu.settle(L.probedSmall, L.small ? 0.97f : 0.92f);
    }
    const bool measuring = !tu.decided && !c->cohTunerMode && sizeKnown;
    int mode = c->cohTunerMode ? c->cohTunerMode : tu.decided ? tu.decided : measuring ? 1 + tu.least_sampled() : 1;
    if (L.probedSmall && mode == 1) mode = 2;
    if (sizeKnown) tu.launches++;
    if (mode == 2) qa.flags |= 32u;
    CohTuner::Pending pe{nullptr, nullptr, mode, q.nRays};
    if (measuring && tu.pending.size() < 16) {
        if (hipEventCreate(&pe.e0) != hipSuccess || hipEventCreate(&pe.e1) != hipSuccess || hipEventRecord(pe.e0, c->stream) != hipSuccess) {
            if (pe.e0) hipEventDestroy(pe.e0);
            if (pe.e1) hipEventDestroy(pe.e1);
            pe.e0 = pe.e1 = nullptr; (void)hipGetLastError();
        }
    }
    if (mode == 3) launch_cwbvh_packet(L.any, s->nodes, s->tris, qa, c->status, L.blocks, c->stream);
    else launch_cwbvh(L.any, 0, s->nodes, tris, qa, c->status, mode == 2 ? L.blocksBase : L.blocks, c->stream, 5, L.small, blocks7);
    const hipError_t le = hipGetLastError();
    if (pe.e0) {
        if (le == hipSuccess && hipEventRecord(pe.e1, c->stream) == hipSuccess) tu.pending.push_back(pe);
        else { hipEventDestroy(pe.e0); hipEventDestroy(pe.e1); }
    }
    HIP_TRY(le);
    return 0;
}

static int launchCwbvhKernels(tbvh_scene* s, QueryArgs& q, const CwbvhLaunch& L) {
    tbvh_context* c = s->ctx;
    const bool autoPad = s->variant == 0 && s->cw.padded != nullptr;
    const uint32_t blocks7 = c->gridOverride ? 0xFFFFFFFFu : (uint32_t)c->numCUs * 28u;
    const float4* tris = s->tris;
#ifdef TBVH_EXPERIMENTS
    if ((c->expFlags & 2u) && s->cw.trisPadded) { tris = s->cw.trisPadded; q.flags |= 2u; }
#endif
    const bool twoFlavors = q.probe && s->variant == 0 && ((!autoPad && s->cw.hybrid && s->cw.trisPadded) || L.probedSmall) && !(c->expFlags & 4u);
    if (s->variant == 90 && s->cw.hybrid && s->cw.trisPadded) {
        launch_cwbvh(L.any, 0, s->cw.hybrid, s->cw.trisPadded, q, c->status, L.blocksBase, c->stream, 13, L.small, blocks7);
    } else if (s->variant == 91) {
        QueryArgs qa = q;
        qa.probe = L.probeWords; qa.baseBlocks = 0; qa.flags |= 16u;
        launch_cwbvh(L.any, 0, s->nodes, tris, qa, c->status, L.blocks, c->stream, 5, L.small, blocks7);
    } else if (s->variant == 92) {
        launch_cwbvh_packet(L.any, s->nodes, s->tris, q, c->status, L.blocks, c->stream);
    } else if (twoFlavors) {
        if (int r = launchCoherentFlavor(s, q, L, tris, blocks7)) return r;
        if (L.probedSmall) {
            QueryArgs qp = q;
            qp.probe = nullptr; qp.baseBlocks = 0;
            launch_cwbvh(L.any, s->variant, autoPad ? s->cw.padded : s->nodes, tris, qp, c->status, L.blocks, c->stream, autoPad ? 8 : 5, L.small, blocks7);
        } else {
            uint32_t wX = (c->expFlags >> 8) & 0xffu;
            if (wX > 32u) wX = 32u;
            const uint32_t wB = wX ? wX : (c->gridOverride ? 0u : 28u);
            launch_cwbvh(L.any, 0, s->cw.hybrid, s->cw.trisPadded, q, c->status, (wB && L.blocksBase == c->blocks) ? (uint32_t)c->numCUs * wB : L.blocksBase, c->stream, 13, L.small, blocks7);
        }
    } else {
        launch_cwbvh(L.any, s->variant, autoPad ? s->cw.padded : s->nodes, tris, q, c->status, L.blocks, c->stream, autoPad ? 8 : 5, L.small, blocks7);
    }
    return 0;
}

int launchQuery(tbvh_scene* s, RayRec* d_rays, uint64_t n, uint8_t* d_occ, bool fresh, float freshTmax, const unsigned long long* nDev) {
    tbvh_context* c = s->ctx;
    TBVH_ENTER(c);
    if (n == 0) return 0;
    s->raysTraced += n;
    countQueryForRecopy(s);
    if (!s->isTlas && (nDev || n >= 1024u)) makeCopyOnce(s, kCopyWide8);
    if (tbvh_scene* w = wideCopyForQuery(s)) return launchQuery(w, d_rays, n, d_occ, fresh, freshTmax, nDev);
    const bool any = d_occ != nullptr;
    if (any && s->isTlas && !s->anyHitSeen && !s->blasSpheres) {
        s->anyHitSeen = true;
        for (tbvh_scene* b : s->blasList) makeCopyOnce(b, kCopyWide8);
        if (int r = reclassifyTlas(s)) return r;
    }
    const size_t poolWords = (size_t)(kPoolParts + 1) * kPoolCounterStride;
    if (!c->poolClean) HIP_TRY(hipMemsetAsync(c->pool, 0, poolWords * 4 * 2, c->stream));
    c->poolClean = false;
    uint32_t* const poolArea = (uint32_t*)c->pool + (size_t)c->poolCur * poolWords;
    QueryArgs q;
    q.rays = d_rays; q.nRays = n; q.occluded = d_occ;
    q.spill = c->spill; q.counter = poolArea; q.counterNext = (uint32_t*)c->pool + (size_t)(c->poolCur ^ 1) * poolWords; q.poolParts = c->poolParts;
    q.stats = c->counter + 8;
    q.fresh = fresh ? 1u : 0u; q.freshTmax = freshTmax; q.nRaysDev = nDev; q.omm = Omm{s->opmap, s->opmapN};
    q.probe = nullptr; q.baseBlocks = 0; q.hybridK = s->cw.packed; q.flags = 0u;
#ifdef TBVH_EXPERIMENTS
    q.flags = c->expFlags & 0x3FF0001u;
#endif
    c->lastProbed = false;
    q.splitBelow = c->splitBelow;
    const uint64_t blobBytes = (!s->isTlas && s->layout == TBVH_LAYOUT_CWBVH) ? (s->nNodeBlocks + s->nTriBlocks) * 16 : s->bytes;
    const bool small = !s->isTlas && !c->gridOverride && blobBytes < (48ull << 20);
    const uint32_t perBlock = c->raysPerBlock;
    const uint32_t cap = small ? c->blocks + c->blocks / 3u : c->blocks;
    uint64_t want = (n + perBlock - 1) / perBlock;
    const uint32_t lo = (uint32_t)c->numCUs * 4u;
    uint32_t blocks = (uint32_t)(want < lo ? lo : (want > cap ? cap : want));
    const bool probed = !s->isTlas && !small && blobBytes <= (384ull << 20) && s->layout == TBVH_LAYOUT_CWBVH && n >= (1ull << 21) && (s->variant == 0 || s->variant == 88) && !(c->expFlags & 64u);
    if (probed) { if (int r = prepareIncoherentCopies(s)) return r; }
    q.hybridK = s->cw.packed;
    HIP_TRY(timedBegin(c));
    uint32_t blocksBase = blocks;
    const bool huge = !small && blobBytes > (384ull << 20);
    const int sizeClass = (small && n < (3ull << 19)) ? 3 : n < (6ull << 20) ? 0 : n < (12ull << 20) ? 1 : 2;
    bool probedSmall = !s->isTlas && (small || huge) && s->layout == TBVH_LAYOUT_CWBVH && s->variant == 0 && !nDev && n >= (small ? (3ull << 18) : (6ull << 20)) && !(c->expFlags & 64u) && !c->gridOverride;
    if (probedSmall) {
        const int m = c->cohTunerMode ? c->cohTunerMode : s->cohTuner[any ? 1 : 0][sizeClass].decided;
        if (m == 1 || m == 2) { probedSmall = false; s->cohLastClass[any ? 1 : 0] = (uint8_t)sizeClass; }
    }
    if (probedSmall) {
        q.probe = poolArea + (size_t)kPoolParts * kPoolCounterStride; q.baseBlocks = blocks;
        c->lastProbed = true;
    }
    if (probed) {
        uint32_t* probe = poolArea + (size_t)kPoolParts * kPoolCounterStride;
        q.probe = probe; q.baseBlocks = blocks;
        c->lastProbed = true;
        if (!c->gridOverride && blocks == c->blocks) blocks = c->blocks + c->blocks / 3u;
    }
    if (s->isTlas) {
        launchTlasKernels(s, q, any, blocks);
        HIP_TRY(hipGetLastError());
        HIP_TRY(timedEnd(c));
        c->poolCur ^= 1; c->poolClean = true;
        return 0;
    }
    switch (s->layout) {
    case TBVH_LAYOUT_BVH_GPU:
        q.spillStride = c->spillEntries;
        launch_bvh2(any, s->variant, s->nodes, s->tris, q, c->status, blocks, c->stream);
        break;
    case TBVH_LAYOUT_BVH4_GPU:
        q.spillStride = c->spillEntries;
        launch_bvh4(any, s->variant, s->nodes, q, c->status, blocks, c->stream);
        break;
    case TBVH_LAYOUT_CWBVH:
        q.spillStride = c->spillEntries / 2;
        if (int r = launchCwbvhKernels(s, q, CwbvhLaunch{any, small, probedSmall, sizeClass, blocks, blocksBase, poolArea + (size_t)kPoolParts * kPoolCounterStride})) return r;
        break;
    case TBVH_LAYOUT_BVH2_WALD:
        q.spillStride = c->spillEntries / 2;
        launch_custom(any, s->nodes, s->tris, q, c->status, blocks, c->stream);
        break;
    case TBVH_LAYOUT_VOXELSET:
        q.spillStride = c->spillEntries;
        launch_voxel(any, (const uint32_t*)s->nodes.get(), nullptr, nullptr, nullptr, nullptr, q, c->status, blocks, c->stream);
        break;
    default:
        return fail(TBVH_E_INVALID, "scene layout %d has no query kernel", s->layout);
    }
    HIP_TRY(hipGetLastError());
    HIP_TRY(timedEnd(c));
    c->poolCur ^= 1; c->poolClean = true;
    return 0;
}

int checkStatus(tbvh_context* c) {
    uint32_t st = 0;
    HIP_TRY(hipMemcpyAsync(&st, c->status, 4, hipMemcpyDeviceToHost, c->stream));
    HIP_TRY(hipStreamSynchronize(c->stream));
    if (st & 1u) {
        hipMemsetAsync(c->status, 0, 4, c->stream);
        return fail(TBVH_E_FORMAT, "traversal stack overflow (tree deeper than the spill area allows)");
    }
    if (st & 2u) {
        hipMemsetAsync(c->status, 0, 4, c->stream);
        return fail(TBVH_E_FORMAT, "refit: a triangle record refers to a primitive beyond the vertex array");
    }
    if (st & 4u) {
        hipMemsetAsync(c->status, 0, 4, c->stream);
        return fail(TBVH_E_FORMAT, "wide TLAS build: the node capacity did not hold the collapsed tree");
    }
    if (st & 16u) {
        hipMemsetAsync(c->status, 0, 4, c->stream);
        return fail(TBVH_E_FORMAT, "sphere query: a triangle record refers to a primitive beyond the vertex array");
    }
    if (st & kStatusMeshIndex) {
        hipMemsetAsync(c->status, 0, 4, c->stream);
        return fail(TBVH_E_FORMAT, "mesh: a vertex index of a device-resident index buffer is not a vertex (index >= n_verts)");
    }
    if (st & kStatusPoseJoint) {
        hipMemsetAsync(c->status, 0, 4, c->stream);
        return fail(TBVH_E_FORMAT, "pose: a joint index of a device-resident joint array is not a joint (index >= n_joints); that vertex was not written");
    }
    if (st & kStatusOmmIndex) {
        hipMemsetAsync(c->status, 0, 4, c->stream);
        return fail(TBVH_E_FORMAT, "opacity micromap bake: a device-resident index is not a UV (>= n_uv; clamped) or a texture index is not a texture (>= n_textures; taken as none)");
    }
    if (st & kStatusGraph) {
        hipMemsetAsync(c->status, 0, 4, c->stream);
        return fail(TBVH_E_FORMAT, "scene graph: a sampler, node, key state or key position of a graph was out of range on the device; that channel, node, instance or joint was not written");
    }
    if (st & kStatusShade) {
        hipMemsetAsync(c->status, 0, 4, c->stream);
        return fail(TBVH_E_FORMAT, "shade: a hit record's instance, BLAS slot or primitive, or a device-resident material or texture index, is out of range (the record got no surface, or an untextured albedo of 0)");
    }
    return 0;
}
}

extern "C" {


int tbvh_intersect_device(tbvh_scene* s, void* dRays, uint64_t n) {
    TBVH_REFUSE_DOUBLE(s, "tbvh_intersect_device");
    if (!s || (!dRays && n)) return fail(TBVH_E_INVALID, "tbvh_intersect_device: null argument");
    if (((uintptr_t)dRays) & 15) return fail(TBVH_E_INVALID, "ray array must be 16-byte aligned");
    return launchQuery(s, (RayRec*)dRays, n, nullptr);
}

int tbvh_intersect_device_fresh(tbvh_scene* s, void* dRays, uint64_t n, float tmax) {
    TBVH_REFUSE_DOUBLE(s, "tbvh_intersect_device_fresh");
    if (!s || (!dRays && n)) return fail(TBVH_E_INVALID, "tbvh_intersect_device_fresh: null argument");
    if (((uintptr_t)dRays) & 15) return fail(TBVH_E_INVALID, "ray array must be 16-byte aligned");
    return launchQuery(s, (RayRec*)dRays, n, nullptr, true, tmax);
}

int tbvh_occluded_device(tbvh_scene* s, const void* dRays, uint64_t n, uint8_t* dOcc) {
    TBVH_REFUSE_DOUBLE(s, "tbvh_occluded_device");
    if (!s || ((!dRays || !dOcc) && n)) return fail(TBVH_E_INVALID, "tbvh_occluded_device: null argument");
    if (((uintptr_t)dRays) & 15) return fail(TBVH_E_INVALID, "ray array must be 16-byte aligned");
    return launchQuery(s, (RayRec*)dRays, n, dOcc);
}

int tbvh_intersect(tbvh_scene* s, void* rays, uint64_t n, uint32_t stride) {
    TBVH_REFUSE_DOUBLE(s, "tbvh_intersect");
    if (!s || (!rays && n)) return fail(TBVH_E_INVALID, "tbvh_intersect: null argument");
    if (stride < 64 || (stride & 3)) return fail(TBVH_E_INVALID, "stride must be >= 64 and a multiple of 4 (got %u)", stride);
    if (n == 0) return 0;
    tbvh_context* c = s->ctx;
    TBVH_ENTER(c);
    return hostQuery(s, (const char*)rays, (char*)rays, n, stride, nullptr);
}

int tbvh_occluded(tbvh_scene* s, const void* rays, uint64_t n, uint32_t stride, uint8_t* occ) {
    TBVH_REFUSE_DOUBLE(s, "tbvh_occluded");
    if (!s || ((!rays || !occ) && n)) return fail(TBVH_E_INVALID, "tbvh_occluded: null argument");
    if (stride < 64 || (stride & 3)) return fail(TBVH_E_INVALID, "stride must be >= 64 and a multiple of 4 (got %u)", stride);
    if (n == 0) return 0;
    tbvh_context* c = s->ctx;
    TBVH_ENTER(c);
    return hostQuery(s, (const char*)rays, nullptr, n, stride, occ);
}

int tbvh_pinned_malloc(tbvh_context* c, uint64_t bytes, void** out) {
    if (!c || !out || !bytes) return fail(TBVH_E_INVALID, "tbvh_pinned_malloc: null/empty argument");
    TBVH_ENTER(c);
    void* p = nullptr;
    if (hipHostMalloc(&p, bytes, hipHostMallocPortable) != hipSuccess || !p) { (void)hipGetLastError(); return fail(TBVH_E_NOMEM, "tbvh_pinned_malloc: cannot page-lock %llu bytes", (unsigned long long)bytes); }
    try { c->pinned.push_back(tbvh_context::PinnedRange{(char*)p, bytes}); }
    catch (const std::bad_alloc&) { hipHostFree(p); return fail(TBVH_E_NOMEM, "out of host memory"); }
    *out = p;
    return 0;
}

int tbvh_pinned_free(tbvh_context* c, void* ptr) {
    if (!c || !ptr) return fail(TBVH_E_INVALID, "tbvh_pinned_free: null argument");
    TBVH_ENTER(c);
    for (size_t i = 0; i < c->pinned.size(); i++)
        if (c->pinned[i].host == (char*)ptr) {
            HIP_TRY(hipStreamSynchronize(c->stream));
            c->pinned.erase(c->pinned.begin() + i);
            HIP_TRY(hipHostFree(ptr));
            return 0;
        }
    return fail(TBVH_E_INVALID, "tbvh_pinned_free: %p did not come from tbvh_pinned_malloc of this context", ptr);
}

void tbvh_shard_range(uint64_t n_rays, uint32_t rank, uint32_t world, uint64_t* begin, uint64_t* end) {
    const uint64_t align = 64, units = (n_rays + align - 1) / align;
    const uint64_t base = world ? units / world : 0, extra = world ? units % world : 0;
    const uint64_t b = (uint64_t)rank * base + (rank < extra ? rank : extra), e = b + base + (rank < extra ? 1 : 0);
    if (begin) *begin = b * align < n_rays ? b * align : n_rays;
    if (end) *end = e * align < n_rays ? e * align : n_rays;
}

namespace {
int shardedQuery(tbvh_scene* const* scenes, uint32_t nDev, void* rays, uint64_t n, uint32_t stride, uint8_t* occ, const char* who) {
    if (!scenes || nDev == 0 || (!rays && n)) return fail(TBVH_E_INVALID, "%s: null/empty argument", who);
    if (stride < 64 || (stride & 3)) return fail(TBVH_E_INVALID, "stride must be >= 64 and a multiple of 4 (got %u)", stride);
    for (uint32_t i = 0; i < nDev; i++) {
        if (!scenes[i]) return fail(TBVH_E_INVALID, "%s: scene %u is null", who, i);
        TBVH_REFUSE_DOUBLE(scenes[i], who);
        if (scenes[i]->layout != scenes[0]->layout || scenes[i]->isTlas != scenes[0]->isTlas) return fail(TBVH_E_INVALID, "%s: scene %u is not a replica of scene 0 (layout differs)", who, i);
        for (uint32_t j = 0; j < i; j++) if (scenes[j]->ctx == scenes[i]->ctx) return fail(TBVH_E_INVALID, "%s: scenes %u and %u share a context (one context, i.e. one stream and staging area, per shard)", who, j, i);
    }
    if (n == 0) return 0;
    std::vector<int> rc(nDev, 0);
    std::vector<std::string> msg(nDev);
    auto work = [&](uint32_t i) {
        uint64_t b, e;
        tbvh_shard_range(n, i, nDev, &b, &e);
        if (e == b) return;
        char* base = (char*)rays + b * stride;
        rc[i] = occ ? tbvh_occluded(scenes[i], base, e - b, stride, occ + b) : tbvh_intersect(scenes[i], base, e - b, stride);
        if (rc[i]) msg[i] = tbvh_last_error();
    };
    std::vector<std::thread> th;
    for (uint32_t i = 1; i < nDev; i++) th.emplace_back(work, i);
    work(0);
    for (auto& t : th) t.join();
    for (uint32_t i = 0; i < nDev; i++) if (rc[i]) return fail(rc[i], "%s: shard %u (device %d): %s", who, i, scenes[i]->ctx->device, msg[i].c_str());
    return 0;
}
}
// ... 120 lines not shown
```

### tinybvh_amd/csrc/capi_scene.hip

```cpp
#include "capi_internal.h"

using namespace tbvh;
using namespace tbvh_capi;

namespace tbvh_capi {
tbvh_scene* newScene(tbvh_context* c, int layout) {
    tbvh_scene* s = new (std::nothrow) tbvh_scene;
    if (!s) return nullptr;
    s->ctx = c; s->layout = layout;
    c->scenes.push_back(s);
    return s;
}

int refitDeviceSource(tbvh_scene* s, const MeshSrc& src) {
    tbvh_context* c = s->ctx;
    if (s->layout == TBVH_LAYOUT_BVH4_GPU) {
        const uint32_t capNodes = (uint32_t)(s->nNodeBlocks / 4 + 1);
        if (!s->refitScratch) HIP_TRY(s->refitScratch.alloc((size_t)capNodes * (16 + 128) + 256));
        char* base = (char*)s->refitScratch.get();
        uint32_t* counter = (uint32_t*)base;
        void* items = base + 256;
        float4* childBox = (float4*)(base + 256 + (size_t)capNodes * 16);
        HIP_TRY(timedBegin(c));
        HIP_TRY(run_refit_bvh4(s->nodes, s->nNodeBlocks, src, items, capNodes, counter, childBox, s->b4Levels, c->status, c->stream));
// ... 629 lines not shown
    src.nTris = mesh->n_tris; src.nVerts = (uint32_t)mesh->n_verts; src.stride = mesh->stride_bytes ? mesh->stride_bytes : 16u;
    src.verts = (const float4*)mesh->verts;
    if (!mesh->on_device) {
        if (int r = stageRefitVertices(s, mesh->verts, meshVertexBytes(*mesh))) return r;
        src.verts = (const float4*)s->vertStage.get();
    }
    if (!mesh->indices) {
        src.indices = held ? s->meshIdx : nullptr;
        return refitDeviceSource(s, src);
    }
    DevBuf<uint32_t> tmp;
    src.indices = mesh->indices;
    if (!mesh->on_device) {
        HIP_TRY(tmp.alloc(mesh->n_tris * 3));
        if (hipMemcpyAsync(tmp, mesh->indices, mesh->n_tris * 12, hipMemcpyHostToDevice, c->stream) != hipSuccess) return fail(TBVH_E_HIP, "tbvh_refit_mesh: copying the indices failed");
        src.indices = tmp;
    }
    int r = refitDeviceSource(s, src);
    if (!r && mesh->on_device) r = checkStatus(c);
    if (!r && s->meshIdx) r = keepMeshIndices(s, src);
    if (tmp) hipStreamSynchronize(c->stream);
    return r;
}

int tbvh_rebuild_tlas_device(tbvh_scene* s, const void* transforms, int onDevice, const float* blasBounds6, uint64_t nBlas) {
    TBVH_REFUSE_DOUBLE(s, "tbvh_rebuild_tlas_device");
    if (!s || !s->isTlas) return fail(TBVH_E_INVALID, "tbvh_rebuild_tlas_device: not a TLAS");
    tbvh_context* c = s->ctx;
    TBVH_ENTER(c);
    const uint64_t n = s->nInst;
    if (n == 0 || n > 0x7fffffffull) return fail(TBVH_E_INVALID, "tbvh_rebuild_tlas_device: %llu instances", (unsigned long long)n);
    if (blasBounds6) {
        if (nBlas != s->nBlas) return fail(TBVH_E_INVALID, "tbvh_rebuild_tlas_device: %llu BLAS bounds for a TLAS over %llu BLASes", (unsigned long long)nBlas, (unsigned long long)s->nBlas);
        if (!s->blasBounds) HIP_TRY(s->blasBounds.alloc(s->nBlas * 6));
        HIP_TRY(hipMemcpyAsync(s->blasBounds, blasBounds6, s->nBlas * 24, hipMemcpyHostToDevice, c->stream));
        HIP_TRY(hipStreamSynchronize(c->stream));
    }
    if (!s->blasBounds) return fail(TBVH_E_INVALID, "tbvh_rebuild_tlas_device: the first call needs blas_bounds6");
    const uint64_t nNodes = 2 * n - 1;
    HIP_TRY(s->nodes.reserve(nNodes * 4));
    HIP_TRY(s->tlasIdx.reserve(n));
    if (s->buildScratchFor != n) {
        s->buildScratchFor = 0;
        HIP_TRY(s->buildScratch.alloc(tlas_build_scratch_bytes((uint32_t)n, &s->sortTempBytes)));
        s->buildScratchFor = n;
    }
    const float* xf = nullptr;
    if (transforms) {
        if (onDevice) xf = (const float*)transforms;
        else {
            HIP_TRY(s->xformStage.reserve(n * 16));
            HIP_TRY(hipMemcpyAsync(s->xformStage, transforms, n * 64, hipMemcpyHostToDevice, c->stream));
            xf = s->xformStage;
        }
    }
    HIP_TRY(timedBegin(c));
    HIP_TRY(launch_tlas_rebuild(s->nodes, s->tlasIdx, s->instances, xf, s->blasBounds, (uint32_t)n, (uint32_t)s->nBlas, s->buildScratch, s->sortTempBytes, c->stream));
    s->bytes = nNodes * 64 + n * 4 + n * 192;
    s->nTlasNodes = nNodes; s->nTlasIdx = n;
    if (int r = buildTlas4(s)) return r;
    HIP_TRY(timedEnd(c));
    return 0;
}

int tbvh_tlas_download(tbvh_scene* s, void* nodes64, uint64_t capNodes, uint32_t* idx, uint64_t capIdx, void* instances192, uint64_t capInst,
                       uint64_t* nNodesOut) {
    TBVH_REFUSE_DOUBLE(s, "tbvh_tlas_download");
    if (!s || !s->isTlas) return fail(TBVH_E_INVALID, "tbvh_tlas_download: not a TLAS");
    tbvh_context* c = s->ctx;
    TBVH_ENTER(c);
    HIP_TRY(hipStreamSynchronize(c->stream));
    const uint64_t n = s->nInst, nNodes = s->nTlasNodes;
    if (nNodesOut) *nNodesOut = nNodes;
    if (nodes64) { if (capNodes < nNodes) return fail(TBVH_E_INVALID, "tbvh_tlas_download: node buffer too small"); HIP_TRY(hipMemcpy(nodes64, s->nodes, nNodes * 64, hipMemcpyDeviceToHost)); }
    if (idx) { if (capIdx < n) return fail(TBVH_E_INVALID, "tbvh_tlas_download: index buffer too small"); HIP_TRY(hipMemcpy(idx, s->tlasIdx, n * 4, hipMemcpyDeviceToHost)); }
    if (instances192) { if (capInst < n) return fail(TBVH_E_INVALID, "tbvh_tlas_download: instance buffer too small"); HIP_TRY(hipMemcpy(instances192, s->instances, n * 192, hipMemcpyDeviceToHost)); }
    return 0;
}

void tbvh_free_scene(tbvh_scene* s) {
    if (!s) return;
    tbvh_context* c = s->ctx;
    TBVH_LOCK(c);
    hipSetDevice(c->device);
    hipStreamSynchronize(c->stream);
    if (!s->isTlas && !s->usedBy.empty()) { s->zombie = true; return; }
    freeCopy(s, kCopyWide8);
    freeCopy(s, kCopyWide4);
    if (s->isTlas) {
        std::vector<tbvh_scene*> mine;
        mine.swap(s->blasList);
        for (tbvh_scene* b : mine) {
            for (size_t i = 0; i < b->usedBy.size(); i++) if (b->usedBy[i] == s) { b->usedBy.erase(b->usedBy.begin() + i); break; }
            if (b->zombie && b->usedBy.empty()) { b->zombie = false; tbvh_free_scene(b); }
        }
    }
    for (auto& kind : s->cohTuner) for (CohTuner& tu : kind) tu.drop_pending();
    for (size_t i = 0; i < c->scenes.size(); i++)
        if (c->scenes[i] == s) { c->scenes.erase(c->scenes.begin() + i); break; }
    delete s;
}
int tbvh_scene_layout(const tbvh_scene* s) { return s ? s->layout : TBVH_E_INVALID; }
uint64_t tbvh_scene_device_bytes(const tbvh_scene* s) { return s ? s->bytes : 0; }

int tbvh_debug_coherent_schedule(tbvh_scene* s, int anyhit, uint32_t out[4]) {
    if (!s || !out) return fail(TBVH_E_INVALID, "tbvh_debug_coherent_schedule: null argument");
    TBVH_LOCK(s->ctx);
    s = tunedScene(s);
    const CohTuner& t = s->cohTuner[anyhit ? 1 : 0][s->cohLastClass[anyhit ? 1 : 0]];
    out[0] = s->ctx->cohTunerMode ? (uint32_t)s->ctx->cohTunerMode : (uint32_t)t.decided;
    out[1] = t.n[0]; out[2] = t.n[1];
    out[3] = (t.n[0] && t.n[1]) ? (uint32_t)(1000.f * t.best[1] / t.best[0]) : 0u;
    return 0;
}

int tbvh_scene_get_schedule_hint(tbvh_scene* s, tbvh_schedule_hint* out) {
    TBVH_REFUSE_DOUBLE(s, "tbvh_scene_get_schedule_hint");
    TBVH_REFUSE_VOXEL(s, "tbvh_scene_get_schedule_hint");
    TBVH_REFUSE_CUSTOM(s, "tbvh_scene_get_schedule_hint");
    if (!s || !out) return fail(TBVH_E_INVALID, "tbvh_scene_get_schedule_hint: null argument");
    TBVH_LOCK(s->ctx);
    std::memset(out, 0, sizeof *out);
    s = tunedScene(s);
    for (int k = 0; k < 3; k++) {
        out->closest_hit[k] = (uint8_t)(s->ctx->cohTunerMode ? s->ctx->cohTunerMode : s->cohTuner[0][k].decided);
        out->any_hit[k] = (uint8_t)(s->ctx->cohTunerMode ? s->ctx->cohTunerMode : s->cohTuner[1][k].decided);
    }
    out->reserved[0] = (uint8_t)(s->ctx->cohTunerMode ? s->ctx->cohTunerMode : s->cohTuner[0][3].decided);
    out->reserved[1] = (uint8_t)(s->ctx->cohTunerMode ? s->ctx->cohTunerMode : s->cohTuner[1][3].decided);
    return 0;
}

int tbvh_scene_set_schedule_hint(tbvh_scene* s, const tbvh_schedule_hint* hint) {
    TBVH_REFUSE_DOUBLE(s, "tbvh_scene_set_schedule_hint");
    TBVH_REFUSE_VOXEL(s, "tbvh_scene_set_schedule_hint");
    TBVH_REFUSE_CUSTOM(s, "tbvh_scene_set_schedule_hint");
    if (!s || !hint) return fail(TBVH_E_INVALID, "tbvh_scene_set_schedule_hint: null argument");
    for (int k = 0; k < 3; k++) if (hint->closest_hit[k] > 3 || hint->any_hit[k] > 3) return fail(TBVH_E_INVALID, "tbvh_scene_set_schedule_hint: entries are 0 (measure), 1 (deferred + gated), 2 (strict) or 3 (one traversal per wave)");
    if (hint->reserved[0] > 3 || hint->reserved[1] > 3) return fail(TBVH_E_INVALID, "tbvh_scene_set_schedule_hint: entries are 0 (measure), 1 (deferred + gated), 2 (strict) or 3 (one traversal per wave)");
    TBVH_LOCK(s->ctx);
    s = tunedScene(s);
    for (int a = 0; a < 2; a++) for (int k = 0; k < 4; k++) {
        const uint8_t v = k == 3 ? hint->reserved[a] : a ? hint->any_hit[k] : hint->closest_hit[k];
        CohTuner& tu = s->cohTuner[a][k];
        tu.drop_pending();
        tu = CohTuner();
        if (v) { tu.decided = v; tu.pinned = true; }
    }
    return 0;
}

int tbvh_set_variant(tbvh_scene* s, int v) {
    if (!s) return fail(TBVH_E_INVALID, "null scene");
    TBVH_LOCK(s->ctx);
    const bool ok = v == 0 || (!s->isTlas && s->layout == TBVH_LAYOUT_CWBVH && cwbvh_variant_valid(v)) || (!s->isTlas && (s->layout == TBVH_LAYOUT_BVH_GPU || s->layout == TBVH_LAYOUT_BVH4_GPU) && v == 1);
    if (!ok) return fail(TBVH_E_INVALID, "unknown variant %d for layout %d", v, s->layout);
    const bool viewChanges = !s->isTlas && s->copies.live() && (s->variant == 0) != (v == 0);
    s->variant = v;
    if (viewChanges) return refreshBlasDescs(s);
    return 0;
}
}
```

### tinybvh_amd/csrc/capi_scenegraph.hip

```cpp
#include "capi_internal.h"
#include "scenegraph_host.h"
#include "../../include/tinybvh_amd_debug.h"

using namespace tbvh;
using namespace tbvh_capi;

struct tbvh_scenegraph {
    tbvh_context* ctx = nullptr;
    SgCompiled c;
    DevBuf<char> mem;
    SgView view;
    float* combinedBuf[2] = {nullptr, nullptr};
    int cur = 0;
};

namespace {

struct Packer {
    std::vector<char> bytes;
    template <class T>
    size_t put(const std::vector<T>& v, size_t minCount = 1) {
        const size_t at = (bytes.size() + 255) & ~(size_t)255;
        bytes.resize(at + std::max(v.size(), minCount) * sizeof(T), 0);
        if (!v.empty()) memcpy(bytes.data() + at, v.data(), v.size() * sizeof(T));
// ... 135 lines not shown
    return 0;
}

int tbvh_scenegraph_instance_transforms(tbvh_scenegraph* g, const float** dMats16, uint64_t* n) {
    if (!g || !dMats16) return fail(TBVH_E_INVALID, "tbvh_scenegraph_instance_transforms: null argument");
    *dMats16 = g->view.instOut;
    if (n) *n = g->c.nInstances;
    return 0;
}

int tbvh_scenegraph_joint_matrices(tbvh_scenegraph* g, uint32_t use, const float** dMats16, uint32_t* n) {
    if (!g || !dMats16) return fail(TBVH_E_INVALID, "tbvh_scenegraph_joint_matrices: null argument");
    if (use >= g->c.nUses) return fail(TBVH_E_INVALID, "tbvh_scenegraph_joint_matrices: skin use %u of %u", use, g->c.nUses);
    *dMats16 = g->view.jointOut + (size_t)g->c.useOff[use] * 16;
    if (n) *n = g->c.useOff[use + 1] - g->c.useOff[use];
    return 0;
}

int tbvh_scenegraph_morph_weights(tbvh_scenegraph* g, uint32_t node, const float** dWeights, uint32_t* n) {
    if (!g || !dWeights) return fail(TBVH_E_INVALID, "tbvh_scenegraph_morph_weights: null argument");
    if (node >= g->c.nNodes) return fail(TBVH_E_INVALID, "tbvh_scenegraph_morph_weights: node %u of %u", node, g->c.nNodes);
    *dWeights = g->view.weights + g->c.wOff[node];
    if (n) *n = g->c.wOff[node + 1] - g->c.wOff[node];
    return 0;
}

namespace {
const void* arrayOf(const tbvh_scenegraph* g, int what) {
    const SgView& v = g->view;
    switch (what) {
    case TBVH_GRAPH_TRS: return v.trs;
    case TBVH_GRAPH_LOCAL: return v.local;
    case TBVH_GRAPH_COMBINED: return g->combinedBuf[g->cur];
    case TBVH_GRAPH_CHANNEL_T: return v.cT;
    case TBVH_GRAPH_CHANNEL_K: return v.cK;
    case TBVH_GRAPH_INSTANCES: return v.instOut;
    case TBVH_GRAPH_JOINTS: return v.jointOut;
    case TBVH_GRAPH_WEIGHTS: return v.weights;
    case TBVH_GRAPH_STALE: return v.pairStale;
    case TBVH_GRAPH_TRIG: return v.cTrig;
    }
    return nullptr;
}
}

int tbvh_debug_scenegraph_array(tbvh_scenegraph* g, int what, void** dPtr) {
    if (!g || !dPtr) return fail(TBVH_E_INVALID, "tbvh_debug_scenegraph_array: null argument");
    if (!(*dPtr = const_cast<void*>(arrayOf(g, what)))) return fail(TBVH_E_INVALID, "tbvh_debug_scenegraph_array: what = %d", what);
    return 0;
}

int tbvh_debug_scenegraph_step(tbvh_scenegraph* g, int step, float dt) {
    if (!g || step < 0 || step > 3) return fail(TBVH_E_INVALID, "tbvh_debug_scenegraph_step: null graph or step %d", step);
    if (int r = sg_check_time(g->c, "tbvh_debug_scenegraph_step", dt)) return r;
    tbvh_context* c = g->ctx;
    TBVH_ENTER(c);
    HIP_TRY(timedBegin(c));
    if (step == 0) launch_graph_sample(g->view, 0, g->c.nChannels, dt, kSgShadowAll, c->stream);
    else {
        if (step == 2) { g->cur ^= 1; setCombined(g); }
        launch_graph_walk(g->view, step, c->stream);
    }
    HIP_TRY(hipGetLastError());
    HIP_TRY(timedEnd(c));
    return 0;
}

int tbvh_scenegraph_download(tbvh_scenegraph* g, int what, void* dst, uint64_t cap) {
    if (!g || !dst) return fail(TBVH_E_INVALID, "tbvh_scenegraph_download: null argument");
    const void* src = arrayOf(g, what);
    if (!src) return fail(TBVH_E_INVALID, "tbvh_scenegraph_download: what = %d", what);
    const uint64_t bytes = sg_download_bytes(g->c, what);
    if (cap < bytes) return fail(TBVH_E_INVALID, "tbvh_scenegraph_download: room for %llu bytes, %llu needed", (unsigned long long)cap, (unsigned long long)bytes);
    tbvh_context* c = g->ctx;
    TBVH_ENTER(c);
    if (bytes) HIP_TRY(hipMemcpyAsync(dst, src, bytes, hipMemcpyDeviceToHost, c->stream));
    return checkStatus(c);
}

void tbvh_scenegraph_free(tbvh_scenegraph* g) {
    if (!g) return;
    tbvh_context* c = g->ctx;
    TBVH_LOCK(c);
    hipSetDevice(c->device);
    hipStreamSynchronize(c->stream);
    for (size_t i = 0; i < c->graphs.size(); i++)
        if (c->graphs[i] == g) { c->graphs.erase(c->graphs.begin() + i); break; }
    delete g;
}

}
```

### tinybvh_amd/csrc/capi_shade.hip

```cpp
#include "capi_internal.h"
#include "shade.h"

#include <stddef.h>

using namespace tbvh;
using namespace tbvh_capi;

struct FatTriCheck {
    float u0, u1, u2; int32_t ltriIdx;
    float v0, v1, v2; uint32_t material;
    float vN0[3], Nx, vN1[3], Ny, vN2[3], Nz;
    float vertex0[3], u0_2, vertex1[3], u1_2, vertex2[3], u2_2;
    float T[3], area, B[3], invArea;
    float alpha[3], LOD, v0_2, v1_2, v2_2, dummy4;
};
static_assert(sizeof(FatTriCheck) == 192 && sizeof(FatTriCheck) == kFatTriQuads * 16, "FatTri is 192 bytes");
static_assert(offsetof(FatTriCheck, u0) == 0 && offsetof(FatTriCheck, v0) == 16 && offsetof(FatTriCheck, material) == 28, "FatTri: q0 = u0 u1 u2 ., q1 = v0 v1 v2 material");
static_assert(offsetof(FatTriCheck, vN0) == 32 && offsetof(FatTriCheck, Nx) == 44 && offsetof(FatTriCheck, vN1) == 48 && offsetof(FatTriCheck, Ny) == 60 &&
              offsetof(FatTriCheck, vN2) == 64 && offsetof(FatTriCheck, Nz) == 76, "FatTri: q2..q4 = vN0 Nx, vN1 Ny, vN2 Nz");
static_assert(offsetof(FatTriCheck, vertex0) == 80 && offsetof(FatTriCheck, vertex1) == 96 && offsetof(FatTriCheck, vertex2) == 112, "FatTri: q5..q7 = the vertices");
static_assert(offsetof(FatTriCheck, T) == 128 && offsetof(FatTriCheck, B) == 144, "FatTri: q8 = T area, q9 = B invArea");
static_assert(offsetof(BLASInstanceCheck, blasIdx) == 35 * 4, "BLASInstance: transform rows in float4 0..3, blasIdx at dword 35");
static_assert(sizeof(ShadeMat) == sizeof(tbvh_material) && offsetof(ShadeMat, colorTex) == offsetof(tbvh_material, color_texture) &&
              offsetof(ShadeMat, normalTex) == offsetof(tbvh_material, normal_texture), "ShadeMat is tbvh_material");
// ... 72 lines not shown

extern "C" {

int tbvh_shading_create(tbvh_context* c, const tbvh_material* materials, uint32_t nMats, const tbvh_alpha_texture* textures, uint32_t nTex, int onDevice, tbvh_shading** out) {
    if (!c || !out) return fail(TBVH_E_INVALID, "tbvh_shading_create: null argument");
    if (int r = checkTables("tbvh_shading_create", materials, nMats, textures, nTex, !onDevice, 3)) return r;
    TBVH_ENTER(c);
    tbvh_shading* sh = new (std::nothrow) tbvh_shading;
    if (!sh) return fail(TBVH_E_NOMEM, "tbvh_shading_create: out of host memory");
    sh->ctx = c; sh->nMats = nMats; sh->nTex = nTex;
    std::vector<ShadeTex> desc(nTex);
    int r = 0;
    if (sh->mats.alloc(nMats) != hipSuccess || (nTex && sh->tex.alloc(nTex) != hipSuccess)) r = allocFail("tbvh_shading_create", nMats * sizeof(ShadeMat) + nTex * sizeof(ShadeTex));
    if (!r && !onDevice) sh->texels.resize(nTex);
    for (uint32_t k = 0; k < nTex && !r; k++) {
        desc[k] = ShadeTex{textures[k].texels, textures[k].width, textures[k].height};
        if (onDevice) continue;
        const uint64_t n = (uint64_t)desc[k].width * desc[k].height;
        if (sh->texels[k].alloc(n) != hipSuccess) { r = allocFail("tbvh_shading_create", n * 4); break; }
        if (hipMemcpyAsync(sh->texels[k], desc[k].texels, n * 4, hipMemcpyHostToDevice, c->stream) != hipSuccess) r = fail(TBVH_E_HIP, "tbvh_shading_create: copying texture %u failed: %s", k, hipGetErrorString(hipGetLastError()));
        desc[k].texels = sh->texels[k];
    }
    if (!r && (hipMemcpyAsync(sh->mats, materials, nMats * sizeof(ShadeMat), onDevice ? hipMemcpyDeviceToDevice : hipMemcpyHostToDevice, c->stream) != hipSuccess ||
               (nTex && hipMemcpyAsync(sh->tex, desc.data(), nTex * sizeof(ShadeTex), hipMemcpyHostToDevice, c->stream) != hipSuccess)))
        r = fail(TBVH_E_HIP, "tbvh_shading_create: copying the tables failed: %s", hipGetErrorString(hipGetLastError()));
    const hipError_t e = hipStreamSynchronize(c->stream);
    if (!r && e != hipSuccess) r = fail(TBVH_E_HIP, "tbvh_shading_create: %s", hipGetErrorString(e));
    if (r) { destroyShading(sh); return r; }
    c->shadings.push_back(sh);
    *out = sh;
    return 0;
}

int tbvh_shading_set_fat_tris(tbvh_shading* sh, uint32_t slot, const void* fatTris192, uint64_t nTris, int onDevice) {
    if (!sh || !fatTris192) return fail(TBVH_E_INVALID, "tbvh_shading_set_fat_tris: null argument");
    if (nTris == 0 || nTris >> 32) return fail(TBVH_E_INVALID, "tbvh_shading_set_fat_tris: %llu triangles", (unsigned long long)nTris);
    if (slot >= (1u << 24)) return fail(TBVH_E_INVALID, "tbvh_shading_set_fat_tris: BLAS slot %u (below 2^24)", slot);
    if ((uintptr_t)fatTris192 & (onDevice ? 15 : 3)) return fail(TBVH_E_INVALID, "tbvh_shading_set_fat_tris: misaligned records (device: 16 bytes, host: 4)");
    if (!onDevice)
        if (int r = checkFatTris("tbvh_shading_set_fat_tris", slot, fatTris192, nTris, sh->nMats)) return r;
    tbvh_context* c = sh->ctx;
    TBVH_ENTER(c);
    DevBuf<float4> fresh;
    if (fresh.alloc(nTris * kFatTriQuads) != hipSuccess) return allocFail("tbvh_shading_set_fat_tris", nTris * 192);
    std::vector<ShadeSlot> slots = sh->slots;
    if (slot >= slots.size()) slots.resize(slot + 1, ShadeSlot{nullptr, 0});
    slots[slot] = ShadeSlot{fresh.get(), nTris};
    DevBuf<ShadeSlot> table;
    if (table.alloc(slots.size()) != hipSuccess) return allocFail("tbvh_shading_set_fat_tris", slots.size() * sizeof(ShadeSlot));
    HIP_TRY(hipMemcpyAsync(fresh, fatTris192, nTris * 192, onDevice ? hipMemcpyDeviceToDevice : hipMemcpyHostToDevice, c->stream));
    HIP_TRY(hipMemcpyAsync(table, slots.data(), slots.size() * sizeof(ShadeSlot), hipMemcpyHostToDevice, c->stream));
    HIP_TRY(hipStreamSynchronize(c->stream));
    sh->slotsDev = std::move(table);
    if (slot >= sh->tris.size()) sh->tris.resize(slot + 1);
    sh->tris[slot] = std::move(fresh);
    sh->slots.swap(slots);
    return 0;
}

int tbvh_shading_fat_tris(tbvh_shading* sh, uint32_t slot, void** dFatTris192, uint64_t* nTris) {
    if (!sh || !dFatTris192) return fail(TBVH_E_INVALID, "tbvh_shading_fat_tris: null argument");
    TBVH_LOCK(sh->ctx);
    if (slot >= sh->slots.size() || !sh->slots[slot].tris) return fail(TBVH_E_INVALID, "tbvh_shading_fat_tris: slot %u has no records", slot);
    *dFatTris192 = sh->tris[slot].get();
    if (nTris) *nTris = sh->slots[slot].nTris;
    return 0;
}

int tbvh_shading_download_fat_tris(tbvh_shading* sh, uint32_t slot, void* dst192, uint64_t capTris) {
    if (!sh || !dst192) return fail(TBVH_E_INVALID, "tbvh_shading_download_fat_tris: null argument");
    tbvh_context* c = sh->ctx;
    TBVH_ENTER(c);
    if (slot >= sh->slots.size() || !sh->slots[slot].tris) return fail(TBVH_E_INVALID, "tbvh_shading_download_fat_tris: slot %u has no records", slot);
    const uint64_t n = sh->slots[slot].nTris;
    if (capTris < n) return fail(TBVH_E_INVALID, "tbvh_shading_download_fat_tris: room for %llu triangles, the slot has %llu", (unsigned long long)capTris, (unsigned long long)n);
    HIP_TRY(hipMemcpyAsync(dst192, sh->tris[slot], n * 192, hipMemcpyDeviceToHost, c->stream));
    return checkStatus(c);
}

void tbvh_shading_free(tbvh_shading* sh) {
    if (!sh) return;
    tbvh_context* c = sh->ctx;
    TBVH_LOCK(c);
    hipSetDevice(c->device);
    hipStreamSynchronize(c->stream);
    for (size_t i = 0; i < c->shadings.size(); i++)
        if (c->shadings[i] == sh) { c->shadings.erase(c->shadings.begin() + i); break; }
    detachPosesFrom(c, sh);
    destroyShading(sh);
}

int tbvh_shade_hits_device(tbvh_shading* sh, tbvh_scene* s, const void* dRays, uint64_t n, uint32_t strideBytes, void* dOut48) {
    if (!sh || !s) return fail(TBVH_E_INVALID, "tbvh_shade_hits_device: null argument");
    TBVH_REFUSE_DOUBLE(s, "tbvh_shade_hits_device");
    TBVH_REFUSE_VOXEL(s, "tbvh_shade_hits_device");
    TBVH_REFUSE_CUSTOM(s, "tbvh_shade_hits_device");
    if (s->ctx != sh->ctx) return fail(TBVH_E_INVALID, "tbvh_shade_hits_device: the shading table and the scene belong to different contexts");
    if (int r = checkRays("tbvh_shade_hits_device", dRays, n, strideBytes, dOut48)) return r;
    tbvh_context* c = sh->ctx;
    TBVH_ENTER(c);
    if (!n) return 0;
    HIP_TRY(timedBegin(c));
    if (s->isTlas)
        launch_shade_hits(sh->tables(), s->instances, s->nInst, (const uint32_t*)((const char*)s->blasDesc.get() + offsetof(BlasDesc, layout)), sizeof(BlasDesc) / 4,
                          (uint32_t)s->nBlas, dRays, n, strideBytes, dOut48, c->status, c->stream);
    else
        launch_shade_hits(sh->tables(), nullptr, 0, nullptr, 0, 0, dRays, n, strideBytes, dOut48, c->status, c->stream);
    HIP_TRY(hipGetLastError());
    HIP_TRY(timedEnd(c));
    return 0;
}

int tbvh_shade_hits(tbvh_shading* sh, tbvh_scene* s, const void* rays, uint64_t n, uint32_t strideBytes, void* out48) {
    if (!sh || !s) return fail(TBVH_E_INVALID, "tbvh_shade_hits: null argument");
    if (strideBytes < 64 || (strideBytes & 3)) return fail(TBVH_E_INVALID, "tbvh_shade_hits: a record stride of %u bytes (64 or more, a multiple of 4)", strideBytes);
    if (n && (!rays || !out48)) return fail(TBVH_E_INVALID, "tbvh_shade_hits: null records or output");
    if (((uintptr_t)rays | (uintptr_t)out48) & 3) return fail(TBVH_E_INVALID, "tbvh_shade_hits: misaligned records or output (4 bytes)");
    tbvh_context* c = sh->ctx;
    TBVH_ENTER(c);
    if (!n) return 0;
    DevBuf<void> dRays, dOut;
    if (dRays.alloc(n * 64) != hipSuccess || dOut.alloc(n * 48) != hipSuccess) return allocFail("tbvh_shade_hits", n * 112);
    HIP_TRY(hipMemcpy2DAsync(dRays, 64, rays, strideBytes, 64, n, hipMemcpyHostToDevice, c->stream));
    int r = tbvh_shade_hits_device(sh, s, dRays, n, 64, dOut);
    if (!r && hipMemcpyAsync(out48, dOut, n * 48, hipMemcpyDeviceToHost, c->stream) != hipSuccess) r = fail(TBVH_E_HIP, "tbvh_shade_hits: copying the records back failed: %s", hipGetErrorString(hipGetLastError()));
    const int st = checkStatus(c);
    return r ? r : st;
}

int tbvh_shade_continue_device(tbvh_context* c, void* dRays, uint32_t strideBytes, const void* dOut48, uint64_t n, unsigned long long* dContinued) {
    if (!c) return fail(TBVH_E_INVALID, "tbvh_shade_continue_device: null context");
    if (int r = checkRays("tbvh_shade_continue_device", dRays, n, strideBytes, dOut48)) return r;
    if ((uintptr_t)dContinued & 7) return fail(TBVH_E_INVALID, "tbvh_shade_continue_device: misaligned counter (8 bytes)");
    TBVH_ENTER(c);
    launch_shade_continue(dRays, strideBytes, dOut48, n, dContinued, c->stream);
    HIP_TRY(hipGetLastError());
    return 0;
}

int tbvh_host_shade_hits(const tbvh_material* materials, uint32_t nMats, const tbvh_alpha_texture* textures, uint32_t nTex, const void* const* fatTris192,
                         const uint64_t* nTris, uint32_t nSlots, const void* instances192, uint64_t nInst, const void* rays, uint64_t n, uint32_t strideBytes,
                         void* out48) {
    if (int r = checkTables("tbvh_host_shade_hits", materials, nMats, textures, nTex, true, 3)) return r;
    if (!fatTris192 || !nTris || nSlots == 0) return fail(TBVH_E_INVALID, "tbvh_host_shade_hits: no BLAS slots");
    if (int r = checkRays("tbvh_host_shade_hits", rays, n, strideBytes, out48)) return r;
    if ((uintptr_t)instances192 & 15) return fail(TBVH_E_INVALID, "tbvh_host_shade_hits: misaligned instance records (16 bytes)");
    if (instances192 && nInst == 0) return fail(TBVH_E_INVALID, "tbvh_host_shade_hits: an instance array without instances");
    std::vector<ShadeSlot> slots(nSlots);
    for (uint32_t k = 0; k < nSlots; k++) {
        if (!fatTris192[k] != !nTris[k] || nTris[k] >> 32) return fail(TBVH_E_INVALID, "tbvh_host_shade_hits: slot %u: %llu triangles at %p", k, (unsigned long long)nTris[k], fatTris192[k]);
        if ((uintptr_t)fatTris192[k] & 15) return fail(TBVH_E_INVALID, "tbvh_host_shade_hits: slot %u: misaligned records (16 bytes)", k);
        if (int r = checkFatTris("tbvh_host_shade_hits", k, fatTris192[k], nTris[k], nMats)) return r;
        slots[k] = ShadeSlot{(const float4*)fatTris192[k], nTris[k]};
    }
    const ShadeTables tb{slots.data(), (const ShadeMat*)materials, (const ShadeTex*)textures, nSlots, nMats, nTex};
    bool ok = true;
    for (uint64_t i = 0; i < n; i++) {
        const float4* rec = (const float4*)((const char*)rays + i * strideBytes);
        uint32_t inst;
        memcpy(&inst, &rec[2].w, 4);
        ok &= shade_hit(tb, (const float4*)instances192, nInst, nullptr, 0, 0, rec[1], inst, rec[3], (float4*)out48 + 3 * i);
    }
    return ok ? 0 : fail(TBVH_E_FORMAT, "tbvh_host_shade_hits: a hit record's instance, BLAS slot or primitive is out of range (the record got no surface)");
}

}
```

### tinybvh_amd/csrc/capi_wavefront.hip

```cpp
#include "capi_internal.h"

using namespace tbvh;
using namespace tbvh_capi;

extern "C" {


constexpr uint32_t kWfCounterWords = 32u * 18u;

struct tbvh_wavefront {
    tbvh_context* ctx = nullptr;
    uint32_t width = 0, height = 0;
    uint32_t firstRow = 0, fullHeight = 0;
    uint64_t n = 0;
    DevBuf<RayRec> rays[2];
    DevBuf<PathAux> aux[2];
    DevBuf<RayRec> shadow;
    DevBuf<PathAux> shadowAux;
    DevBuf<uint8_t> occ;
    DevBuf<float> accum;
    DevBuf<const float4*> blasVerts;
    uint64_t nBlasVerts = 0;
    DevBuf<uint32_t> blueNoise;
    DevBuf<unsigned long long> counters;
    hipEvent_t e0 = nullptr, e1 = nullptr;
};

int tbvh_wavefront_create(tbvh_context* c, uint32_t width, uint32_t height, tbvh_wavefront** out) {
    if (!c || !out || !width || !height || (width & 3) || (height & 3)) return fail(TBVH_E_INVALID, "tbvh_wavefront_create: null argument or size not a multiple of 4");
    TBVH_ENTER(c);
    tbvh_wavefront* w = new (std::nothrow) tbvh_wavefront;
    if (!w) return fail(TBVH_E_NOMEM, "out of host memory");
    w->ctx = c; w->width = width; w->height = height; w->n = (uint64_t)width * height;
    hipError_t e = hipSuccess;
    for (int i = 0; i < 2 && e == hipSuccess; i++) {
        e = w->rays[i].alloc(w->n);
        if (e == hipSuccess) e = w->aux[i].alloc(w->n);
    }
    if (e == hipSuccess) e = w->shadow.alloc(w->n);
    if (e == hipSuccess) e = w->shadowAux.alloc(w->n);
    if (e == hipSuccess) e = w->occ.alloc(w->n);
    if (e == hipSuccess) e = w->accum.alloc(w->n * 4);
    if (e == hipSuccess) e = w->counters.alloc(kWfCounterWords);
    if (e == hipSuccess) e = hipMemset(w->accum, 0, w->n * 16);
    if (e == hipSuccess) e = hipEventCreate(&w->e0);
    if (e == hipSuccess) e = hipEventCreate(&w->e1);
    if (e != hipSuccess) { tbvh_wavefront_destroy(w); return fail(TBVH_E_NOMEM, "wavefront allocation failed: %s", hipGetErrorString(e)); }
    *out = w;
    return 0;
}

void tbvh_wavefront_destroy(tbvh_wavefront* w) {
    if (!w) return;
    TBVH_LOCK(w->ctx);
    hipSetDevice(w->ctx->device);
    hipStreamSynchronize(w->ctx->stream);
    if (w->ctx->ev0 == w->e0 || w->ctx->ev1 == w->e1) { w->ctx->timed = false; w->ctx->ev0 = w->ctx->ev1 = nullptr; }
    if (w->e0) hipEventDestroy(w->e0);
    if (w->e1) hipEventDestroy(w->e1);
    delete w;
}

int tbvh_wavefront_set_blas_vertices(tbvh_wavefront* w, const void* const* dVertsPerBlas, uint64_t nBlas) {
    if (!w || !dVertsPerBlas || !nBlas) return fail(TBVH_E_INVALID, "tbvh_wavefront_set_blas_vertices: null/empty argument");
    TBVH_ENTER(w->ctx);
    HIP_TRY(hipStreamSynchronize(w->ctx->stream));
    w->nBlasVerts = 0;
    HIP_TRY(w->blasVerts.alloc(nBlas));
    HIP_TRY(hipMemcpy(w->blasVerts, dVertsPerBlas, nBlas * sizeof(void*), hipMemcpyHostToDevice));
    w->nBlasVerts = nBlas;
    return 0;
}

int tbvh_wavefront_render(tbvh_wavefront* w, tbvh_scene* scene, const void* dVerts, const tbvh_camera* cam, const tbvh_wf_params* p,
                          tbvh_wf_stats* stats) {
    TBVH_REFUSE_DOUBLE(scene, "tbvh_wavefront_render");
    TBVH_REFUSE_VOXEL(scene, "tbvh_wavefront_render");
    TBVH_REFUSE_CUSTOM(scene, "tbvh_wavefront_render");
    if (scene && scene->isTlas && scene->blasSpheres)
        return fail(TBVH_E_INVALID, "tbvh_wavefront_render: a TLAS with sphere BLASes (custom geometry) takes the queries only (the path tracer shades triangles)");
    if (scene && scene->isTlas && !scene->blasList.empty() && scene->blasList[0]->layout == TBVH_LAYOUT_VOXELSET)
        return fail(TBVH_E_INVALID, "tbvh_wavefront_render: a TLAS over VOXELSET scenes takes the queries only (the path tracer shades triangles)");
    if (!w || !scene || !cam || !p) return fail(TBVH_E_INVALID, "tbvh_wavefront_render: null argument");
    if (scene->isTlas) {
        if (w->nBlasVerts < scene->nBlas) return fail(TBVH_E_INVALID, "tbvh_wavefront_render: a TLAS scene needs tbvh_wavefront_set_blas_vertices (%llu BLASes)", (unsigned long long)scene->nBlas);
    } else if (!dVerts) return fail(TBVH_E_INVALID, "tbvh_wavefront_render: null vertex array");
    if (scene->ctx != w->ctx) return fail(TBVH_E_INVALID, "scene and wavefront belong to different contexts");
    const uint32_t fullH = w->fullHeight ? w->fullHeight : w->height;
    if (cam->width != w->width || cam->height != fullH) return fail(TBVH_E_INVALID, "camera size differs from the wavefront's (a band takes the FULL image's camera)");
    const uint32_t maxDepth = p->max_depth ? (p->max_depth > 8 ? 8 : p->max_depth) : 3;
    tbvh_context* c = w->ctx;
    TBVH_ENTER(c);
    hipStream_t st = c->stream;
    HIP_TRY(hipEventRecord(w->e0, st));
    if (p->clear) HIP_TRY(hipMemsetAsync(w->accum, 0, w->n * 16, st));
    auto QP = [&](uint32_t d) { return &w->counters[32u * d]; };
    auto QS = [&](uint32_t d) { return &w->counters[32u * (9u + d)]; };
    CameraArgs ca;
    memcpy(ca.eye, cam->eye, 12); memcpy(ca.p1, cam->p1, 12); memcpy(ca.p2, cam->p2, 12); memcpy(ca.p3, cam->p3, 12);
    ca.width = cam->width; ca.height = cam->height; ca.sppX = ca.sppY = 1;
    launch_wf_generate(ca, w->rays[0], w->aux[0], w->n, p->seed, w->firstRow, w->height, w->counters, kWfCounterWords, st);
    int cur = 0;
    struct Untimed { tbvh_context* c; bool was; ~Untimed() { c->skipTiming = was; } } untimed{c, c->skipTiming};
    c->skipTiming = true;
    for (uint32_t d = 0; d < maxDepth; d++) {
        const int nxt = cur ^ 1;
        if (int r = launchQuery(scene, w->rays[cur], w->n, nullptr, false, 1e30f, d == 0 ? nullptr : QP(d))) return r;
        ShadeArgs a;
        a.in = w->rays[cur]; a.auxIn = w->aux[cur]; a.nIn = QP(d);
        a.out = w->rays[nxt]; a.auxOut = w->aux[nxt]; a.nOut = QP(d + 1);
        a.shadow = w->shadow; a.shadowAux = w->shadowAux; a.nShadow = QS(d);
        a.verts = (const float4*)dVerts; a.accum = w->accum;
        a.blasVerts = scene->isTlas ? w->blasVerts : nullptr; a.instances = scene->isTlas ? scene->instances : nullptr;
        a.blueNoise = w->blueNoise; a.sampleIdx = p->sample_index; a.width = w->width; a.height = fullH; a.pixelOffset = w->firstRow * w->width;
        memcpy(a.lightPos, p->light_pos, 12); memcpy(a.lightColor, p->light_color, 12); memcpy(a.skyLo, p->sky_lo, 12); memcpy(a.skyHi, p->sky_hi, 12);
        a.lightSize[0] = p->light_size[0]; a.lightSize[1] = p->light_size[1]; a.flags = p->flags;
        a.eps = p->eps; a.depth = d; a.maxDepth = maxDepth; a.seed = p->seed;
        launch_wf_shade(a, w->n, st);
        if (int r = launchQuery(scene, w->shadow, w->n, w->occ, false, 1e30f, QS(d))) return r;
        launch_wf_connect(w->occ, w->shadowAux, QS(d), w->accum, w->n, st);
        cur = nxt;
    }
    HIP_TRY(hipGetLastError());
    HIP_TRY(hipEventRecord(w->e1, st));
    c->ev0 = w->e0; c->ev1 = w->e1; c->timed = true;
    if (stats) {
        std::vector<unsigned long long> h(kWfCounterWords);
        HIP_TRY(hipMemcpyAsync(h.data(), w->counters, (size_t)kWfCounterWords * 8, hipMemcpyDeviceToHost, st));
        HIP_TRY(hipStreamSynchronize(st));
        memset(stats, 0, sizeof *stats);
        for (uint32_t d = 0; d < maxDepth; d++) { stats->extend_rays[d] = h[32u * d]; stats->shadow_rays[d] = h[32u * (9u + d)]; }
        HIP_TRY(hipEventElapsedTime(&stats->frame_ms, w->e0, w->e1));
        if (int r = checkStatus(c)) return r;
    }
    return 0;
}

int tbvh_wavefront_set_band(tbvh_wavefront* w, uint32_t firstRow, uint32_t fullHeight) {
// ... 96 lines not shown
```

Measured before the change: 4950 MRays/s.

## Overlap independent device queries on a second stream lane

Adds a second HIP stream with its own ray-pool buffers and a bookkeeping structure that tracks the ray and occlusion byte ranges of in-flight launches. Independent intersect and occluded device queries whose buffers do not overlap alternate between the two streams, so consecutive kernels (for example primary and diffuse batches) can run concurrently. Any API call that needs ordered results joins the lanes through an event wait. Timing is reworked to subtract time overlapped with chained launches. This adds complexity, extra memory for a second pool, and a risk of the two kernels contending for the same compute units rather than gaining from concurrency.

```diff
diff --git a/include/tinybvh_amd.h b/include/tinybvh_amd.h
--- a/include/tinybvh_amd.h
+++ b/include/tinybvh_amd.h
@@ -35,6 +35,7 @@
 void        tbvh_shutdown(tbvh_context* ctx);
 int         tbvh_synchronize(tbvh_context* ctx);
 int         tbvh_set_stream(tbvh_context* ctx, void* hip_stream);
+int         tbvh_context_set_overlap(tbvh_context* ctx, int enabled);
 int         tbvh_set_timing(tbvh_context* ctx, int enabled);
 
 
diff --git a/include/tinybvh_amd_debug.h b/include/tinybvh_amd_debug.h
--- a/include/tinybvh_amd_debug.h
+++ b/include/tinybvh_amd_debug.h
@@ -12,6 +12,9 @@
 int tbvh_debug_coherent_schedule(tbvh_scene* scene, int anyhit, uint32_t out[4]);
 
 int tbvh_debug_last_probe(tbvh_context* ctx, uint32_t out[3]);
+
+int tbvh_debug_overlap_stats(tbvh_context* ctx, uint64_t out[2]);
+int tbvh_debug_lane_script(const uint64_t* ops5, uint64_t n_ops, int32_t* out);
 
 int tbvh_set_variant(tbvh_scene* scene, int variant);
 
diff --git a/tinybvh_amd/__init__.py b/tinybvh_amd/__init__.py
--- a/tinybvh_amd/__init__.py
+++ b/tinybvh_amd/__init__.py
@@ -81,6 +81,14 @@
 
     def set_stream(self, hip_stream: Optional[int]):
         check(lib.tbvh_set_stream(self._h, C.c_void_p(hip_stream or 0)), "tbvh_set_stream")
+
+    def set_overlap(self, enabled: bool):
+        check(lib.tbvh_context_set_overlap(self._h, 1 if enabled else 0), "tbvh_context_set_overlap")
+
+    def overlap_stats(self):
+        out = (C.c_uint64 * 2)()
+        check(lib.tbvh_debug_overlap_stats(self._h, out), "tbvh_debug_overlap_stats")
+        return int(out[0]), int(out[1])
 
     def set_timing(self, enabled: bool):
         check(lib.tbvh_set_timing(self._h, 1 if enabled else 0), "tbvh_set_timing")
diff --git a/tinybvh_amd/_capi.py b/tinybvh_amd/_capi.py
--- a/tinybvh_amd/_capi.py
+++ b/tinybvh_amd/_capi.py
@@ -68,6 +68,9 @@
     "tbvh_shutdown": (None, [_vp]),
     "tbvh_synchronize": (_i, [_vp]),
     "tbvh_set_stream": (_i, [_vp, _vp]),
+    "tbvh_context_set_overlap": (_i, [_vp, _i]),
+    "tbvh_debug_overlap_stats": (_i, [_vp, _vp]),
+    "tbvh_debug_lane_script": (_i, [_vp, _u64, _vp]),
     "tbvh_set_timing": (_i, [_vp, _i]),
     "tbvh_upload_bvh_gpu": (_i, [_vp, _vp, _u64, _vp, _u64, _vp, _u64, _pp]),
     "tbvh_upload_bvh4_gpu": (_i, [_vp, _vp, _u64, _pp]),
diff --git a/tinybvh_amd/csrc/capi_context.hip b/tinybvh_amd/csrc/capi_context.hip
--- a/tinybvh_amd/csrc/capi_context.hip
+++ b/tinybvh_amd/csrc/capi_context.hip
@@ -16,25 +16,59 @@
     return code;
 }
 
+int joinLanes(tbvh_context* c) {
+    if (c->lane1Dirty) {
+        HIP_TRY(hipStreamWaitEvent(c->stream, c->lane1Last, 0));
+        c->lane1Dirty = false;
+        c->laneJoins++;
+    }
+    c->book.joined();
+    c->lane0Touched = true;
+    c->chain++;
+    if (!c->chain) c->chain = 1;
+    return 0;
+}
 int setDevice(tbvh_context* c) {
     HIP_TRY(hipSetDevice(c->device));
-    return 0;
-}
-hipError_t timedBegin(tbvh_context* c) {
+    return joinLanes(c);
+}
+hipError_t timedBegin(tbvh_context* c, hipStream_t lane) {
     if (c->skipTiming) return hipSuccess;
     const uint32_t slot = (uint32_t)(c->evSeq % tbvh_context::kTimeRing);
     for (int k = 0; k < 2; k++)
         if (!c->evRing[slot][k]) { const hipError_t e = hipEventCreate(&c->evRing[slot][k]); if (e != hipSuccess) return e; }
     c->evDone[slot] = false;
+    c->evChain[slot] = 0;
     c->ev0 = c->evRing[slot][0]; c->ev1 = c->evRing[slot][1];
     c->evSeq++;
-    return hipEventRecord(c->ev0, c->stream);
-}
-hipError_t timedEnd(tbvh_context* c) {
+    return hipEventRecord(c->ev0, lane ? lane : c->stream);
+}
+hipError_t timedEnd(tbvh_context* c, hipStream_t lane) {
     if (c->skipTiming) return hipSuccess;
-    const hipError_t e = hipEventRecord(c->ev1, c->stream);
+    const hipError_t e = hipEventRecord(c->ev1, lane ? lane : c->stream);
     if (e == hipSuccess && c->evSeq) { c->evDone[(c->evSeq - 1) % tbvh_context::kTimeRing] = true; c->timed = true; }
     return e;
+}
+float timedMs(tbvh_context* c, uint64_t seq) {
+    constexpr uint64_t R = tbvh_context::kTimeRing;
+    const uint32_t slot = (uint32_t)(seq % R);
+    float own = -1.0f;
+    if (hipEventElapsedTime(&own, c->evRing[slot][0], c->evRing[slot][1]) != hipSuccess) { (void)hipGetLastError(); return -1.0f; }
+    const uint32_t chain = c->evChain[slot];
+    if (!chain) return own;
+    constexpr uint64_t kReach = 2 * LaneBook::kMaxInFlight;
+    const uint64_t oldest = c->evSeq > R ? c->evSeq - R : 0;
+    const uint64_t lo = seq > oldest + kReach ? seq - kReach : oldest, hi = seq + kReach < c->evSeq ? seq + kReach + 1 : c->evSeq;
+    float from = 0.f;
+    for (uint64_t j = lo; j < hi; j++) {
+        const uint32_t sj = (uint32_t)(j % R);
+        if (j == seq || c->evChain[sj] != chain || !c->evDone[sj]) continue;
+        float endJ = 0.f;
+        if (hipEventSynchronize(c->evRing[sj][1]) != hipSuccess || hipEventElapsedTime(&endJ, c->evRing[slot][0], c->evRing[sj][1]) != hipSuccess) { (void)hipGetLastError(); continue; }
+        const bool before = endJ < own || (endJ == own && j < seq);
+        if (before && endJ > from) from = endJ;
+    }
+    return own - from;
 }
 }
 
@@ -80,6 +114,7 @@
     if (const char* e = getenv("TBVH_EMBED_TRIS")) { if (atoi(e) == 0) c->embedTris = false; }
     if (const char* e = getenv("TBVH_DEBUG_FLAGS")) c->expFlags = (uint32_t)strtoul(e, nullptr, 0);
     if (const char* e = getenv("TBVH_COHERENT_TUNER")) { const int v = atoi(e); c->cohTunerMode = v == 0 ? 1 : (v == 2 ? 2 : (v == 3 ? 3 : 0)); }
+    if (const char* e = getenv("TBVH_OVERLAP")) { if (atoi(e) == 0) c->overlap = false; }
     if (const char* e = getenv("TBVH_POOL_PARTS")) {
         const int b = atoi(e);
         if (b >= 0 && (1 << b) <= kPoolParts) c->poolParts = (uint32_t)b;
@@ -103,7 +138,9 @@
 void tbvh_shutdown(tbvh_context* c) {
     if (!c) return;
     hipSetDevice(c->device);
+    if (c->lane1.stream) hipStreamSynchronize(c->lane1.stream);
     if (c->ownStream) hipStreamSynchronize(c->ownStream);
+    c->lane1Dirty = false;
     for (;;) {
         tbvh_scene* t = nullptr;
         for (tbvh_scene* s : c->scenes) if (s->isTlas) { t = s; break; }
@@ -119,6 +156,8 @@
     c->pinned.clear();
     delete c->pipe;
     for (auto& pair : c->evRing) for (hipEvent_t ev : pair) if (ev) hipEventDestroy(ev);
+    if (c->evBase) hipEventDestroy(c->evBase);
+    if (c->lane1.stream) hipStreamDestroy(c->lane1.stream);
     if (c->ownStream) hipStreamDestroy(c->ownStream);
     delete c;
 }
@@ -138,8 +177,54 @@
 
 int tbvh_set_stream(tbvh_context* c, void* s) {
     if (!c) return fail(TBVH_E_INVALID, "null context");
+    TBVH_ENTER(c);
+    c->stream = s ? (hipStream_t)s : c->ownStream;
+    return 0;
+}
+
+int tbvh_context_set_overlap(tbvh_context* c, int enabled) {
+    if (!c) return fail(TBVH_E_INVALID, "tbvh_context_set_overlap: null context");
+    TBVH_ENTER(c);
+    c->overlap = enabled != 0;
+    return 0;
+}
+
+int tbvh_debug_lane_script(const uint64_t* ops5, uint64_t nOps, int32_t* out) {
+    if ((!ops5 || !out) && nOps) return fail(TBVH_E_INVALID, "tbvh_debug_lane_script: null argument");
+    LaneBook book;
+    std::vector<uint8_t> done(nOps, 0);
+    bool allowLane1 = true;
+    auto prune = [&] { book.prune([&](int, uint32_t slot) { return done[slot] != 0; }); };
+    for (uint64_t i = 0; i < nOps; i++) {
+        const uint64_t* op = ops5 + i * 5;
+        out[i] = 0;
+        switch (op[0]) {
+        case 0: {
+            LaneFootprint fp;
+            fp.rays.lo = (uintptr_t)op[1]; fp.rays.hi = (uintptr_t)op[2]; fp.occ.lo = (uintptr_t)op[3]; fp.occ.hi = (uintptr_t)op[4];
+            prune();
+            const LaneChoice ch = book.decide(fp, allowLane1);
+            if (ch.join) book.joined();
+            book.add(ch.lane, fp, (uint32_t)i);
+            out[i] = ch.lane + (ch.join ? 2 : 0);
+            break;
+        }
+        case 1:
+            if (op[1] >= nOps) return fail(TBVH_E_INVALID, "tbvh_debug_lane_script: row %llu finishes a row beyond the script", (unsigned long long)i);
+            done[op[1]] = 1;
+            break;
+        case 2: allowLane1 = op[1] != 0; break;
+        case 3: prune(); out[i] = book.count[0] + 256 * book.count[1]; break;
+        default: return fail(TBVH_E_INVALID, "tbvh_debug_lane_script: row %llu has no such operation", (unsigned long long)i);
+        }
+    }
+    return 0;
+}
+
+int tbvh_debug_overlap_stats(tbvh_context* c, uint64_t out[2]) {
+    if (!c || !out) return fail(TBVH_E_INVALID, "tbvh_debug_overlap_stats: null argument");
     TBVH_LOCK(c);
-    c->stream = s ? (hipStream_t)s : c->ownStream;
+    out[0] = c->lane1Launches; out[1] = c->laneJoins;
     return 0;
 }
 
@@ -150,6 +235,7 @@
     if (c->hostQuerySeq == c->evSeq && c->hostQueryMs >= 0.f) return c->hostQueryMs;
     hipSetDevice(c->device);
     if (hipEventSynchronize(c->ev1) != hipSuccess) return -1.0f;
+    if (c->evSeq && c->ev1 == c->evRing[(c->evSeq - 1) % tbvh_context::kTimeRing][1]) return timedMs(c, c->evSeq - 1);
     float ms = -1.0f;
     if (hipEventElapsedTime(&ms, c->ev0, c->ev1) != hipSuccess) return -1.0f;
     return ms;
@@ -166,7 +252,8 @@
         float t = -1.0f;
         if (c->evDone[slot]) {
             HIP_TRY(hipEventSynchronize(c->evRing[slot][1]));
-            HIP_TRY(hipEventElapsedTime(&t, c->evRing[slot][0], c->evRing[slot][1]));
+            t = timedMs(c, c->evSeq - n + i);
+            if (t < 0.f && !c->evChain[slot]) HIP_TRY(hipEventElapsedTime(&t, c->evRing[slot][0], c->evRing[slot][1]));
         }
         ms[i] = t;
     }
@@ -203,7 +290,9 @@
     out[0] = out[1] = out[2] = 0;
     if (!c->lastProbed) return 0;
     HIP_TRY(hipStreamSynchronize(c->stream));
-    HIP_TRY(hipMemcpy(out, (uint32_t*)c->pool + (size_t)(c->poolCur ^ 1) * ((size_t)(kPoolParts + 1) * kPoolCounterStride) + (size_t)kPoolParts * kPoolCounterStride, 8, hipMemcpyDeviceToHost));
+    const uint32_t* pool = c->lastProbedLane ? c->lane1.pool.get() : c->pool.get();
+    const int last = (c->lastProbedLane ? c->lane1.poolCur : c->poolCur) ^ 1;
+    HIP_TRY(hipMemcpy(out, pool + (size_t)last * ((size_t)(kPoolParts + 1) * kPoolCounterStride) + (size_t)kPoolParts * kPoolCounterStride, 8, hipMemcpyDeviceToHost));
     out[2] = (out[1] != 0 && out[0] * 10u >= out[1] * 6u) ? 2u : 1u;
     return 0;
 }
diff --git a/tinybvh_amd/csrc/capi_internal.h b/tinybvh_amd/csrc/capi_internal.h
--- a/tinybvh_amd/csrc/capi_internal.h
+++ b/tinybvh_amd/csrc/capi_internal.h
@@ -24,6 +24,7 @@
 #include "dev_buf.h"
 #include "host_builder.h"
 #include "kernels.h"
+#include "overlap_lanes.h"
 #include "ray_pool.h"
 
 using namespace tbvh;
@@ -94,6 +95,26 @@
     int poolCur = 0;
     bool poolClean = false;
     uint32_t* status = nullptr;
+    struct Lane1 {
+        hipStream_t stream = nullptr;
+        DevBuf<uint32_t> pool, spill;
+        int poolCur = 0;
+        bool poolClean = false;
+        bool unusable = false;
+    } lane1;
+    bool overlap = true;
+    tbvh_capi::LaneBook book;
+    hipEvent_t evBase = nullptr;
+    hipEvent_t lane1Last = nullptr;
+    hipEvent_t laneStart[2] = {nullptr, nullptr};
+    bool lane1Dirty = false;
+    bool lane0Touched = true;
+    bool lane1SawBase = false;
+    bool serialiseNext = false;
+    int lastProbedLane = 0;
+    uint32_t chain = 1;
+    uint32_t evChain[kTimeRing] = {};
+    uint64_t lane1Launches = 0, laneJoins = 0;
     DevBuf<RayRec> stageRays;
     DevBuf<uint8_t> stageOcc;
     struct HostPipe* pipe = nullptr;
@@ -290,10 +311,12 @@
 int setDevice(tbvh_context* c);
 #define TBVH_LOCK(ctxptr) std::lock_guard<std::recursive_mutex> ctx_lock_((ctxptr)->mu)
 #define TBVH_ENTER(ctxptr) std::lock_guard<std::recursive_mutex> ctx_lock_((ctxptr)->mu); if (int r_ = tbvh_capi::setDevice(ctxptr)) return r_
-hipError_t timedBegin(tbvh_context* c);
-hipError_t timedEnd(tbvh_context* c);
+int joinLanes(tbvh_context* c);
+hipError_t timedBegin(tbvh_context* c, hipStream_t lane = nullptr);
+hipError_t timedEnd(tbvh_context* c, hipStream_t lane = nullptr);
+float timedMs(tbvh_context* c, uint64_t seq);
 int launchQuery(tbvh_scene* s, tbvh::RayRec* d_rays, uint64_t n, uint8_t* d_occ, bool fresh = false, float freshTmax = 1e30f,
-                const unsigned long long* nDev = nullptr);
+                const unsigned long long* nDev = nullptr, bool mayOverlap = false);
 int checkStatus(tbvh_context* c);
 int ensureStage(tbvh_context* c, uint64_t n);
 int ensureStageOcc(tbvh_context* c, uint64_t n);
diff --git a/tinybvh_amd/csrc/capi_pose.hip b/tinybvh_amd/csrc/capi_pose.hip
--- a/tinybvh_amd/csrc/capi_pose.hip
+++ b/tinybvh_amd/csrc/capi_pose.hip
@@ -257,7 +257,7 @@
     if (!p) return;
     tbvh_context* c = p->ctx;
     TBVH_LOCK(c);
-    hipSetDevice(c->device);
+    (void)tbvh_capi::setDevice(c);
     hipStreamSynchronize(c->stream);
     for (size_t i = 0; i < c->poses.size(); i++)
         if (c->poses[i] == p) { c->poses.erase(c->poses.begin() + i); break; }
diff --git a/tinybvh_amd/csrc/capi_query.hip b/tinybvh_amd/csrc/capi_query.hip
--- a/tinybvh_amd/csrc/capi_query.hip
+++ b/tinybvh_amd/csrc/capi_query.hip
@@ -175,7 +175,7 @@
 }
 
 
-static void launchTlasKernels(tbvh_scene* s, QueryArgs& q, bool any, uint32_t blocks) {
+static void launchTlasKernels(tbvh_scene* s, QueryArgs& q, bool any, uint32_t blocks, hipStream_t st) {
     tbvh_context* c = s->ctx;
     const uint32_t blocks7 = (!c->gridOverride && blocks == c->blocks) ? (uint32_t)c->numCUs * 28u : blocks;
     const bool own = any && s->blasDescAny != nullptr;
@@ -184,22 +184,22 @@
     const BlasDesc* desc = own ? s->blasDescAny : s->blasDesc;
     if (s->blasSpheres) {
         q.spillStride = c->spillEntries / 2;
-        launch_tlas_custom(any, layout, s->nodes, s->tlasIdx, s->instances, desc, q, c->status, blocks, c->stream);
+        launch_tlas_custom(any, layout, s->nodes, s->tlasIdx, s->instances, desc, q, c->status, blocks, st);
     } else if (s->tlas4 && layout == TBVH_LAYOUT_BVH4_GPU) {
         q.spillStride = c->spillEntries;
-        launch_tlas4(any, 0, s->tlas4, s->instances, desc, q, c->status, blocks, c->stream, blocks7);
+        launch_tlas4(any, 0, s->tlas4, s->instances, desc, q, c->status, blocks, st, blocks7);
     } else if (s->tlas8 && (layout == TBVH_LAYOUT_CWBVH || mix)) {
         q.spillStride = c->spillEntries / 2;
-        launch_tlas8(any, 0, s->tlas8, s->tlas8Refs, s->instances, desc, q, c->status, blocks, c->stream, blocks7, mix);
+        launch_tlas8(any, 0, s->tlas8, s->tlas8Refs, s->instances, desc, q, c->status, blocks, st, blocks7, mix);
     } else if (layout == TBVH_LAYOUT_VOXELSET) {
         q.spillStride = c->spillEntries;
-        launch_voxel(any, nullptr, s->nodes, s->tlasIdx, s->instances, desc, q, c->status, blocks, c->stream);
+        launch_voxel(any, nullptr, s->nodes, s->tlasIdx, s->instances, desc, q, c->status, blocks, st);
     } else if (layout == TBVH_LAYOUT_BVH_GPU) {
         q.spillStride = c->spillEntries;
-        launch_tlas2(any, 0, s->nodes, s->tlasIdx, s->instances, desc, q, c->status, blocks, c->stream, blocks7);
+        launch_tlas2(any, 0, s->nodes, s->tlasIdx, s->instances, desc, q, c->status, blocks, st, blocks7);
     } else {
         q.spillStride = c->spillEntries / 2;
-        launch_tlas(any, layout, s->nodes, s->tlasIdx, s->instances, desc, q, c->status, blocks, c->stream);
+        launch_tlas(any, layout, s->nodes, s->tlasIdx, s->instances, desc, q, c->status, blocks, st);
     }
 }
 
@@ -211,6 +211,7 @@
     uint32_t blocks;
     uint32_t blocksBase;
     uint32_t* probeWords;
+    hipStream_t stream;
 };
 
 static int launchCoherentFlavor(tbvh_scene* s, const QueryArgs& q, const CwbvhLaunch& L, const float4* tris, uint32_t blocks7) {
@@ -233,17 +234,17 @@
     if (mode == 2) qa.flags |= 32u;
     CohTuner::Pending pe{nullptr, nullptr, mode, q.nRays};
     if (measuring && tu.pending.size() < 16) {
-        if (hipEventCreate(&pe.e0) != hipSuccess || hipEventCreate(&pe.e1) != hipSuccess || hipEventRecord(pe.e0, c->stream) != hipSuccess) {
+        if (hipEventCreate(&pe.e0) != hipSuccess || hipEventCreate(&pe.e1) != hipSuccess || hipEventRecord(pe.e0, L.stream) != hipSuccess) {
             if (pe.e0) hipEventDestroy(pe.e0);
             if (pe.e1) hipEventDestroy(pe.e1);
             pe.e0 = pe.e1 = nullptr; (void)hipGetLastError();
         }
     }
-    if (mode == 3) launch_cwbvh_packet(L.any, s->nodes, s->tris, qa, c->status, L.blocks, c->stream);
-    else launch_cwbvh(L.any, 0, s->nodes, tris, qa, c->status, mode == 2 ? L.blocksBase : L.blocks, c->stream, 5, L.small, blocks7);
+    if (mode == 3) launch_cwbvh_packet(L.any, s->nodes, s->tris, qa, c->status, L.blocks, L.stream);
+    else launch_cwbvh(L.any, 0, s->nodes, tris, qa, c->status, mode == 2 ? L.blocksBase : L.blocks, L.stream, 5, L.small, blocks7);
     const hipError_t le = hipGetLastError();
     if (pe.e0) {
-        if (le == hipSuccess && hipEventRecord(pe.e1, c->stream) == hipSuccess) tu.pending.push_back(pe);
+        if (le == hipSuccess && hipEventRecord(pe.e1, L.stream) == hipSuccess) tu.pending.push_back(pe);
         else { hipEventDestroy(pe.e0); hipEventDestroy(pe.e1); }
     }
     HIP_TRY(le);
@@ -260,52 +261,77 @@
 #endif
     const bool twoFlavors = q.probe && s->variant == 0 && ((!autoPad && s->cw.hybrid && s->cw.trisPadded) || L.probedSmall) && !(c->expFlags & 4u);
     if (s->variant == 90 && s->cw.hybrid && s->cw.trisPadded) {
-        launch_cwbvh(L.any, 0, s->cw.hybrid, s->cw.trisPadded, q, c->status, L.blocksBase, c->stream, 13, L.small, blocks7);
+        launch_cwbvh(L.any, 0, s->cw.hybrid, s->cw.trisPadded, q, c->status, L.blocksBase, L.stream, 13, L.small, blocks7);
     } else if (s->variant == 91) {
         QueryArgs qa = q;
         qa.probe = L.probeWords; qa.baseBlocks = 0; qa.flags |= 16u;
-        launch_cwbvh(L.any, 0, s->nodes, tris, qa, c->status, L.blocks, c->stream, 5, L.small, blocks7);
+        launch_cwbvh(L.any, 0, s->nodes, tris, qa, c->status, L.blocks, L.stream, 5, L.small, blocks7);
     } else if (s->variant == 92) {
-        launch_cwbvh_packet(L.any, s->nodes, s->tris, q, c->status, L.blocks, c->stream);
+        launch_cwbvh_packet(L.any, s->nodes, s->tris, q, c->status, L.blocks, L.stream);
     } else if (twoFlavors) {
         if (int r = launchCoherentFlavor(s, q, L, tris, blocks7)) return r;
         if (L.probedSmall) {
             QueryArgs qp = q;
             qp.probe = nullptr; qp.baseBlocks = 0;
-            launch_cwbvh(L.any, s->variant, autoPad ? s->cw.padded : s->nodes, tris, qp, c->status, L.blocks, c->stream, autoPad ? 8 : 5, L.small, blocks7);
+            launch_cwbvh(L.any, s->variant, autoPad ? s->cw.padded : s->nodes, tris, qp, c->status, L.blocks, L.stream, autoPad ? 8 : 5, L.small, blocks7);
         } else {
             uint32_t wX = (c->expFlags >> 8) & 0xffu;
             if (wX > 32u) wX = 32u;
             const uint32_t wB = wX ? wX : (c->gridOverride ? 0u : 28u);
-            launch_cwbvh(L.any, 0, s->cw.hybrid, s->cw.trisPadded, q, c->status, (wB && L.blocksBase == c->blocks) ? (uint32_t)c->numCUs * wB : L.blocksBase, c->stream, 13, L.small, blocks7);
+            launch_cwbvh(L.any, 0, s->cw.hybrid, s->cw.trisPadded, q, c->status, (wB && L.blocksBase == c->blocks) ? (uint32_t)c->numCUs * wB : L.blocksBase, L.stream, 13, L.small, blocks7);
         }
     } else {
-        launch_cwbvh(L.any, s->variant, autoPad ? s->cw.padded : s->nodes, tris, q, c->status, L.blocks, c->stream, autoPad ? 8 : 5, L.small, blocks7);
-    }
-    return 0;
-}
-
-int launchQuery(tbvh_scene* s, RayRec* d_rays, uint64_t n, uint8_t* d_occ, bool fresh, float freshTmax, const unsigned long long* nDev) {
+        launch_cwbvh(L.any, s->variant, autoPad ? s->cw.padded : s->nodes, tris, q, c->status, L.blocks, L.stream, autoPad ? 8 : 5, L.small, blocks7);
+    }
+    return 0;
+}
+
+static bool ensureLane1(tbvh_context* c) {
+    tbvh_context::Lane1& l = c->lane1;
+    if (l.unusable) return false;
+    if (l.stream && l.pool && l.spill && c->evBase) return true;
+    const size_t poolWords = (size_t)(kPoolParts + 1) * kPoolCounterStride;
+    const size_t spillWords = (size_t)(c->blocks + c->blocks / 3u) * 64 * c->spillEntries;
+    if ((!c->evBase && hipEventCreateWithFlags(&c->evBase, hipEventDisableTiming) != hipSuccess) ||
+        (!l.stream && hipStreamCreateWithFlags(&l.stream, hipStreamNonBlocking) != hipSuccess) ||
+        (!l.pool && l.pool.alloc(poolWords * 2) != hipSuccess) || (!l.spill && l.spill.alloc(spillWords) != hipSuccess)) {
+        (void)hipGetLastError();
+        l.pool.reset(); l.spill.reset();
+        l.unusable = true;
+        return false;
+    }
+    l.poolClean = false;
+    return true;
+}
+
+static bool launchPrepares(const tbvh_scene* s, uint64_t n, bool any) {
+    if (s->isTlas) return s->blasRecopyPending || (any && !s->anyHitSeen && !s->blasSpheres);
+    if (s->copies.pending()) return true;
+    return n >= 1024u && s->variant == 0 && !s->copies.tried8 && (s->layout == TBVH_LAYOUT_BVH_GPU || s->layout == TBVH_LAYOUT_BVH4_GPU);
+}
+
+int launchQuery(tbvh_scene* s, RayRec* d_rays, uint64_t n, uint8_t* d_occ, bool fresh, float freshTmax, const unsigned long long* nDev, bool mayOverlap) {
     tbvh_context* c = s->ctx;
-    TBVH_ENTER(c);
+    TBVH_LOCK(c);
+    const bool any = d_occ != nullptr;
+    bool lanes = mayOverlap && c->overlap && c->stream == c->ownStream && !c->skipTiming && !nDev && n != 0;
+    if (lanes && launchPrepares(s, n, any)) lanes = false;
+    if (lanes) HIP_TRY(hipSetDevice(c->device));
+    else if (int r = setDevice(c)) return r;
     if (n == 0) return 0;
     s->raysTraced += n;
     countQueryForRecopy(s);
     if (!s->isTlas && (nDev || n >= 1024u)) makeCopyOnce(s, kCopyWide8);
-    if (tbvh_scene* w = wideCopyForQuery(s)) return launchQuery(w, d_rays, n, d_occ, fresh, freshTmax, nDev);
-    const bool any = d_occ != nullptr;
+    if (tbvh_scene* w = wideCopyForQuery(s)) return launchQuery(w, d_rays, n, d_occ, fresh, freshTmax, nDev, mayOverlap);
     if (any && s->isTlas && !s->anyHitSeen && !s->blasSpheres) {
         s->anyHitSeen = true;
         for (tbvh_scene* b : s->blasList) makeCopyOnce(b, kCopyWide8);
         if (int r = reclassifyTlas(s)) return r;
     }
     const size_t poolWords = (size_t)(kPoolParts + 1) * kPoolCounterStride;
-    if (!c->poolClean) HIP_TRY(hipMemsetAsync(c->pool, 0, poolWords * 4 * 2, c->stream));
-    c->poolClean = false;
-    uint32_t* const poolArea = (uint32_t*)c->pool + (size_t)c->poolCur * poolWords;
     QueryArgs q;
     q.rays = d_rays; q.nRays = n; q.occluded = d_occ;
-    q.spill = c->spill; q.counter = poolArea; q.counterNext = (uint32_t*)c->pool + (size_t)(c->poolCur ^ 1) * poolWords; q.poolParts = c->poolParts;
+    q.poolParts = c->poolParts;
     q.stats = c->counter + 8;
     q.fresh = fresh ? 1u : 0u; q.freshTmax = freshTmax; q.nRaysDev = nDev; q.omm = Omm{s->opmap, s->opmapN};
     q.probe = nullptr; q.baseBlocks = 0; q.hybridK = s->cw.packed; q.flags = 0u;
@@ -322,10 +348,11 @@
     const uint32_t lo = (uint32_t)c->numCUs * 4u;
     uint32_t blocks = (uint32_t)(want < lo ? lo : (want > cap ? cap : want));
     const bool probed = !s->isTlas && !small && blobBytes <= (384ull << 20) && s->layout == TBVH_LAYOUT_CWBVH && n >= (1ull << 21) && (s->variant == 0 || s->variant == 88) && !(c->expFlags & 64u);
-    if (probed) { if (int r = prepareIncoherentCopies(s)) return r; }
+    if (probed && !s->cw.tried) {
+        if (lanes) if (int r = joinLanes(c)) return r;
+        if (int r = prepareIncoherentCopies(s)) return r;
+    }
     q.hybridK = s->cw.packed;
-    HIP_TRY(timedBegin(c));
-    uint32_t blocksBase = blocks;
     const bool huge = !small && blobBytes > (384ull << 20);
     const int sizeClass = (small && n < (3ull << 19)) ? 3 : n < (6ull << 20) ? 0 : n < (12ull << 20) ? 1 : 2;
     bool probedSmall = !s->isTlas && (small || huge) && s->layout == TBVH_LAYOUT_CWBVH && s->variant == 0 && !nDev && n >= (small ? (3ull << 18) : (6ull << 20)) && !(c->expFlags & 64u) && !c->gridOverride;
@@ -333,55 +360,106 @@
         const int m = c->cohTunerMode ? c->cohTunerMode : s->cohTuner[any ? 1 : 0][sizeClass].decided;
         if (m == 1 || m == 2) { probedSmall = false; s->cohLastClass[any ? 1 : 0] = (uint8_t)sizeClass; }
     }
+    int lane = 0;
+    if (lanes) {
+        const bool tunerMeasures = (probed || probedSmall) && !c->cohTunerMode && !s->cohTuner[any ? 1 : 0][sizeClass].decided;
+        const bool haveLane1 = ensureLane1(c);
+        if (tunerMeasures || c->serialiseNext) {
+            if (int r = joinLanes(c)) return r;
+            c->serialiseNext = tunerMeasures;
+        } else {
+            c->book.prune([c](int, uint32_t slot) {
+                const hipError_t qe = hipEventQuery(c->evRing[slot][1]);
+                if (qe != hipSuccess) (void)hipGetLastError();
+                return qe != hipErrorNotReady;
+            });
+            LaneFootprint fp;
+            fp.rays.lo = (uintptr_t)d_rays; fp.rays.hi = fp.rays.lo + (uintptr_t)n * sizeof(RayRec);
+            if (any) { fp.occ.lo = (uintptr_t)d_occ; fp.occ.hi = fp.occ.lo + (uintptr_t)n; }
+            const LaneChoice ch = c->book.decide(fp, haveLane1);
+            if (ch.join) { if (int r = joinLanes(c)) return r; }
+            lane = ch.lane;
+            if (c->lane0Touched && c->evBase) {
+                HIP_TRY(hipEventRecord(c->evBase, c->stream));
+                c->lane0Touched = false; c->lane1SawBase = false;
+            }
+            if (lane == 1 && !c->lane1SawBase) {
+                HIP_TRY(hipStreamWaitEvent(c->lane1.stream, c->evBase, 0));
+                c->lane1SawBase = true;
+            }
+            if (!c->book.idle(lane ^ 1) && c->laneStart[lane ^ 1]) HIP_TRY(hipStreamWaitEvent(lane ? c->lane1.stream : c->stream, c->laneStart[lane ^ 1], 0));
+        }
+    }
+    const hipStream_t st = lane ? c->lane1.stream : c->stream;
+    uint32_t* const pool = lane ? c->lane1.pool.get() : c->pool.get();
+    int& poolCur = lane ? c->lane1.poolCur : c->poolCur;
+    bool& poolClean = lane ? c->lane1.poolClean : c->poolClean;
+    if (!poolClean) HIP_TRY(hipMemsetAsync(pool, 0, poolWords * 4 * 2, st));
+    poolClean = false;
+    uint32_t* const poolArea = pool + (size_t)poolCur * poolWords;
+    q.spill = lane ? c->lane1.spill : c->spill; q.counter = poolArea; q.counterNext = pool + (size_t)(poolCur ^ 1) * poolWords;
+    HIP_TRY(timedBegin(c, st));
+    const uint32_t ringSlot = (uint32_t)((c->evSeq - 1) % tbvh_context::kTimeRing);
+    auto finish = [&]() -> int {
+        HIP_TRY(hipGetLastError());
+        HIP_TRY(timedEnd(c, st));
+        poolCur ^= 1; poolClean = true;
+        if (lanes) {
+            LaneFootprint fp;
+            fp.rays.lo = (uintptr_t)d_rays; fp.rays.hi = fp.rays.lo + (uintptr_t)n * sizeof(RayRec);
+            if (any) { fp.occ.lo = (uintptr_t)d_occ; fp.occ.hi = fp.occ.lo + (uintptr_t)n; }
+            c->book.add(lane, fp, ringSlot);
+            c->evChain[ringSlot] = c->chain;
+            c->laneStart[lane] = c->evRing[ringSlot][0];
+            if (lane) { c->lane1Last = c->evRing[ringSlot][1]; c->lane1Dirty = true; c->lane1Launches++; }
+        }
+        return 0;
+    };
+    uint32_t blocksBase = blocks;
     if (probedSmall) {
         q.probe = poolArea + (size_t)kPoolParts * kPoolCounterStride; q.baseBlocks = blocks;
-        c->lastProbed = true;
+        c->lastProbed = true; c->lastProbedLane = lane;
     }
     if (probed) {
         uint32_t* probe = poolArea + (size_t)kPoolParts * kPoolCounterStride;
         q.probe = probe; q.baseBlocks = blocks;
-        c->lastProbed = true;
+        c->lastProbed = true; c->lastProbedLane = lane;
         if (!c->gridOverride && blocks == c->blocks) blocks = c->blocks + c->blocks / 3u;
     }
     if (s->isTlas) {
-        launchTlasKernels(s, q, any, blocks);
-        HIP_TRY(hipGetLastError());
-        HIP_TRY(timedEnd(c));
-        c->poolCur ^= 1; c->poolClean = true;
-        return 0;
+        launchTlasKernels(s, q, any, blocks, st);
+        return finish();
     }
     switch (s->layout) {
     case TBVH_LAYOUT_BVH_GPU:
         q.spillStride = c->spillEntries;
-        launch_bvh2(any, s->variant, s->nodes, s->tris, q, c->status, blocks, c->stream);
+        launch_bvh2(any, s->variant, s->nodes, s->tris, q, c->status, blocks, st);
         break;
     case TBVH_LAYOUT_BVH4_GPU:
         q.spillStride = c->spillEntries;
-        launch_bvh4(any, s->variant, s->nodes, q, c->status, blocks, c->stream);
+        launch_bvh4(any, s->variant, s->nodes, q, c->status, blocks, st);
         break;
     case TBVH_LAYOUT_CWBVH:
         q.spillStride = c->spillEntries / 2;
-        if (int r = launchCwbvhKernels(s, q, CwbvhLaunch{any, small, probedSmall, sizeClass, blocks, blocksBase, poolArea + (size_t)kPoolParts * kPoolCounterStride})) return r;
+        if (int r = launchCwbvhKernels(s, q, CwbvhLaunch{any, small, probedSmall, sizeClass, blocks, blocksBase, poolArea + (size_t)kPoolParts * kPoolCounterStride, st})) return r;
         break;
     case TBVH_LAYOUT_BVH2_WALD:
         q.spillStride = c->spillEntries / 2;
-        launch_custom(any, s->nodes, s->tris, q, c->status, blocks, c->stream);
+        launch_custom(any, s->nodes, s->tris, q, c->status, blocks, st);
         break;
     case TBVH_LAYOUT_VOXELSET:
         q.spillStride = c->spillEntries;
-        launch_voxel(any, (const uint32_t*)s->nodes.get(), nullptr, nullptr, nullptr, nullptr, q, c->status, blocks, c->stream);
+        launch_voxel(any, (const uint32_t*)s->nodes.get(), nullptr, nullptr, nullptr, nullptr, q, c->status, blocks, st);
         break;
     default:
         return fail(TBVH_E_INVALID, "scene layout %d has no query kernel", s->layout);
     }
-    HIP_TRY(hipGetLastError());
-    HIP_TRY(timedEnd(c));
-    c->poolCur ^= 1; c->poolClean = true;
-    return 0;
+    return finish();
 }
 
 int checkStatus(tbvh_context* c) {
     uint32_t st = 0;
+    if (int r = joinLanes(c)) return r;
     HIP_TRY(hipMemcpyAsync(&st, c->status, 4, hipMemcpyDeviceToHost, c->stream));
     HIP_TRY(hipStreamSynchronize(c->stream));
     if (st & 1u) {
@@ -431,21 +509,21 @@
     TBVH_REFUSE_DOUBLE(s, "tbvh_intersect_device");
     if (!s || (!dRays && n)) return fail(TBVH_E_INVALID, "tbvh_intersect_device: null argument");
     if (((uintptr_t)dRays) & 15) return fail(TBVH_E_INVALID, "ray array must be 16-byte aligned");
-    return launchQuery(s, (RayRec*)dRays, n, nullptr);
+    return launchQuery(s, (RayRec*)dRays, n, nullptr, false, 1e30f, nullptr, true);
 }
 
 int tbvh_intersect_device_fresh(tbvh_scene* s, void* dRays, uint64_t n, float tmax) {
     TBVH_REFUSE_DOUBLE(s, "tbvh_intersect_device_fresh");
     if (!s || (!dRays && n)) return fail(TBVH_E_INVALID, "tbvh_intersect_device_fresh: null argument");
     if (((uintptr_t)dRays) & 15) return fail(TBVH_E_INVALID, "ray array must be 16-byte aligned");
-    return launchQuery(s, (RayRec*)dRays, n, nullptr, true, tmax);
+    return launchQuery(s, (RayRec*)dRays, n, nullptr, true, tmax, nullptr, true);
 }
 
 int tbvh_occluded_device(tbvh_scene* s, const void* dRays, uint64_t n, uint8_t* dOcc) {
     TBVH_REFUSE_DOUBLE(s, "tbvh_occluded_device");
     if (!s || ((!dRays || !dOcc) && n)) return fail(TBVH_E_INVALID, "tbvh_occluded_device: null argument");
     if (((uintptr_t)dRays) & 15) return fail(TBVH_E_INVALID, "ray array must be 16-byte aligned");
-    return launchQuery(s, (RayRec*)dRays, n, dOcc);
+    return launchQuery(s, (RayRec*)dRays, n, dOcc, false, 1e30f, nullptr, true);
 }
 
 int tbvh_intersect(tbvh_scene* s, void* rays, uint64_t n, uint32_t stride) {
diff --git a/tinybvh_amd/csrc/capi_scene.hip b/tinybvh_amd/csrc/capi_scene.hip
--- a/tinybvh_amd/csrc/capi_scene.hip
+++ b/tinybvh_amd/csrc/capi_scene.hip
@@ -735,7 +735,7 @@
     if (!s) return;
     tbvh_context* c = s->ctx;
     TBVH_LOCK(c);
-    hipSetDevice(c->device);
+    (void)tbvh_capi::setDevice(c);
     hipStreamSynchronize(c->stream);
     if (!s->isTlas && !s->usedBy.empty()) { s->zombie = true; return; }
     freeCopy(s, kCopyWide8);
diff --git a/tinybvh_amd/csrc/capi_scenegraph.hip b/tinybvh_amd/csrc/capi_scenegraph.hip
--- a/tinybvh_amd/csrc/capi_scenegraph.hip
+++ b/tinybvh_amd/csrc/capi_scenegraph.hip
@@ -241,7 +241,7 @@
     if (!g) return;
     tbvh_context* c = g->ctx;
     TBVH_LOCK(c);
-    hipSetDevice(c->device);
+    (void)tbvh_capi::setDevice(c);
     hipStreamSynchronize(c->stream);
     for (size_t i = 0; i < c->graphs.size(); i++)
         if (c->graphs[i] == g) { c->graphs.erase(c->graphs.begin() + i); break; }
diff --git a/tinybvh_amd/csrc/capi_shade.hip b/tinybvh_amd/csrc/capi_shade.hip
--- a/tinybvh_amd/csrc/capi_shade.hip
+++ b/tinybvh_amd/csrc/capi_shade.hip
@@ -178,7 +178,7 @@
     if (!sh) return;
     tbvh_context* c = sh->ctx;
     TBVH_LOCK(c);
-    hipSetDevice(c->device);
+    (void)tbvh_capi::setDevice(c);
     hipStreamSynchronize(c->stream);
     for (size_t i = 0; i < c->shadings.size(); i++)
         if (c->shadings[i] == sh) { c->shadings.erase(c->shadings.begin() + i); break; }
diff --git a/tinybvh_amd/csrc/capi_wavefront.hip b/tinybvh_amd/csrc/capi_wavefront.hip
--- a/tinybvh_amd/csrc/capi_wavefront.hip
+++ b/tinybvh_amd/csrc/capi_wavefront.hip
@@ -53,7 +53,7 @@
 void tbvh_wavefront_destroy(tbvh_wavefront* w) {
     if (!w) return;
     TBVH_LOCK(w->ctx);
-    hipSetDevice(w->ctx->device);
+    (void)tbvh_capi::setDevice(w->ctx);
     hipStreamSynchronize(w->ctx->stream);
     if (w->ctx->ev0 == w->e0 || w->ctx->ev1 == w->e1) { w->ctx->timed = false; w->ctx->ev0 = w->ctx->ev1 = nullptr; }
     if (w->e0) hipEventDestroy(w->e0);
diff --git a/tinybvh_amd/csrc/overlap_lanes.h b/tinybvh_amd/csrc/overlap_lanes.h
--- /dev/null
+++ b/tinybvh_amd/csrc/overlap_lanes.h
@@ -0,0 +1,68 @@
+#pragma once
+#include <cstdint>
+
+namespace tbvh_capi {
+
+struct ByteRange {
+    uintptr_t lo = 0, hi = 0;
+    bool empty() const { return hi <= lo; }
+};
+inline bool rangesIntersect(const ByteRange& a, const ByteRange& b) { return !a.empty() && !b.empty() && a.lo < b.hi && b.lo < a.hi; }
+
+struct LaneFootprint {
+    ByteRange rays, occ;
+};
+inline bool footprintsIntersect(const LaneFootprint& a, const LaneFootprint& b) {
+    return rangesIntersect(a.rays, b.rays) || rangesIntersect(a.rays, b.occ) || rangesIntersect(a.occ, b.rays) || rangesIntersect(a.occ, b.occ);
+}
+
+inline bool rangeCovers(const ByteRange& outer, const ByteRange& inner) { return inner.empty() || (!outer.empty() && outer.lo <= inner.lo && inner.hi <= outer.hi); }
+inline bool footprintCovers(const LaneFootprint& outer, const LaneFootprint& inner) { return rangeCovers(outer.rays, inner.rays) && rangeCovers(outer.occ, inner.occ); }
+
+struct LaneChoice {
+    int lane;
+    bool join;
+};
+
+struct LaneBook {
+    static constexpr int kLanes = 2;
+    static constexpr int kMaxInFlight = 8;
+    struct Record { LaneFootprint fp; uint32_t slot; };
+    Record rec[kLanes][kMaxInFlight];
+    int count[kLanes] = {0, 0};
+    int lastLane = 1;
+
+    template <class Done>
+    void prune(Done done) {
+        for (int l = 0; l < kLanes; l++) {
+            int kept = 0;
+            for (int i = 0; i < count[l]; i++)
+                if (!done(l, rec[l][i].slot)) rec[l][kept++] = rec[l][i];
+            count[l] = kept;
+        }
+    }
+    bool conflicts(int lane, const LaneFootprint& fp) const {
+        for (int i = 0; i < count[lane]; i++) if (footprintsIntersect(rec[lane][i].fp, fp)) return true;
+        return false;
+    }
+    LaneChoice decide(const LaneFootprint& fp, bool allowLane1 = true) const {
+        const bool c0 = conflicts(0, fp), c1 = conflicts(1, fp);
+        if (c0 && c1) return LaneChoice{0, true};
+        int lane = c0 ? 0 : c1 ? 1 : (lastLane ^ 1);
+        if (lane == 1 && !allowLane1) { if (c1) return LaneChoice{0, true}; lane = 0; }
+        if (count[lane] >= kMaxInFlight) return LaneChoice{0, true};
+        return LaneChoice{lane, false};
+    }
+    void add(int lane, const LaneFootprint& fp, uint32_t slot) {
+        int kept = 0;
+        for (int i = 0; i < count[lane]; i++)
+            if (!footprintCovers(fp, rec[lane][i].fp)) rec[lane][kept++] = rec[lane][i];
+        count[lane] = kept;
+        if (count[lane] < kMaxInFlight) rec[lane][count[lane]++] = Record{fp, slot};
+        lastLane = lane;
+    }
+    void joined() { count[0] = count[1] = 0; }
+    bool idle(int lane) const { return count[lane] == 0; }
+};
+
+}
```

New measurement: 5226 MRays/s, median of 6. 5.6% higher.
